# alexanderswerdlow/BEVGen

Measured on AMD Instinct MI355X. Metric: multi-view scenes/sec (6x256x256), higher is better.
Workload: dtype f32 (GEMM/conv/attention products as 3 f16 MFMAs on hi/lo splits, fp32 accumulate); 1 GPU; BASELINE configs[1]: Route M MaskGit, 6x256x256, batch 16 scenes/GPU, 18 iterations, + VQGAN decode to uint8; global_batch=16, parallelism=scene-parallel x1 (RCCL gather of uint8 pixels), precision_mode=f16x3

## Files before the change

### bevgen_amd/csrc/attention_split.hip

```cpp
#include <algorithm>

#include "common.h"
#include "kernels.h"
#include "profiler.h"

namespace bevgen {

typedef _Float16 half8 __attribute__((ext_vector_type(8)));
typedef _Float16 half4 __attribute__((ext_vector_type(4)));
typedef _Float16 half2v __attribute__((ext_vector_type(2)));
typedef uint32_t u32x4 __attribute__((ext_vector_type(4)));

constexpr int SKT = 32;
constexpr int SKLD = 72;
constexpr int SVLD = 36;
constexpr float kLo = 2048.f, kLoI = 1.f / 2048.f;
constexpr int PP_PLANE = SKT * SKLD;
static_assert(SKT * SKLD == 64 * SVLD, "K and V^T planes share one LDS stage layout");

#ifndef BEVGEN_ATTN_DIAG
#define BEVGEN_ATTN_DIAG 0
#endif
#ifndef BEVGEN_ATTN_BUF
#define BEVGEN_ATTN_BUF 1
#endif
#ifdef BEVGEN_ATTN_LAB
__device__ unsigned long long g_attn_trace[8 * 16 * 8];
#define PP_STAMP(k) do { if (TRACE && lane == 0 && t < 16) trace_lds[(wave * 16 + t) * 8 + (k)] = __builtin_readcyclecounter(); } while (0)
#else
#define PP_STAMP(k) do { } while (0)
#endif

template <bool TRACE, bool KS = false>
__global__ __launch_bounds__(512) void attention_split_kernel(AttnSplitArgs a) {
    __shared__ __attribute__((aligned(16))) _Float16 lds[2][4][PP_PLANE];
    __shared__ __attribute__((aligned(16))) float ostage[8][32 * 68];
#ifdef BEVGEN_ATTN_LAB
    __shared__ unsigned long long trace_lds[TRACE ? 8 * 16 * 8 : 1];
#endif

    const int tid = threadIdx.x, lane = tid & 63, wave = tid >> 6, grp = wave >> 2;
    const int qi = lane & 31, h = lane >> 5;
    const int nqb = gridDim.x, total = nqb * gridDim.y * gridDim.z;
    const int lin = blockIdx.x + nqb * (blockIdx.y + gridDim.y * blockIdx.z);
    const int vid = (total % 8 == 0) ? (lin % 8) * (total / 8) + lin / 8 : lin;
    const int qblk = vid % nqb, head = (vid / nqb) % gridDim.y, bz = vid / (nqb * gridDim.y);
    const int nks = KS ? a.ksplit : 1;
    const int b = KS ? bz / nks : bz, ks = KS ? bz - b * nks : 0;
    const int qrow = qblk * 256 + wave * 32 + qi;
    const bool qvalid = qrow < a.Nq;
    const int qc = qvalid ? qrow : a.Nq - 1;

    const long qoff = ((long)b * a.H + head) * a.Nq * 64 + (long)qc * 64 + 8 * h;
    const long koff = ((long)(b / a.kv_group) * a.H + head) * (long)a.Nk_pad * 64;
    const int bstep = a.bias_pk_tile_step;
    const int ntiles_all = a.Nk_pad / SKT;
    const int t_first = KS ? ks * ntiles_all / nks : 0;
    const int ntiles = KS ? (ks + 1) * ntiles_all / nks - t_first : ntiles_all;
    const float* Bp = a.bias_pk + (long)head * a.bias_head_stride + (long)(qblk * 8 + wave) * a.bias_pk_qb_stride + lane * 4 + (long)t_first * bstep;

    half8 qh[4], qs[4], qls[4];
#pragma unroll
    for (int s = 0; s < 4; ++s) {
        qh[s] = *reinterpret_cast<const half8*>(a.Qh + qoff + 16 * s);
        const half8 ql = *reinterpret_cast<const half8*>(a.Ql + qoff + 16 * s);
#pragma unroll
        for (int e = 0; e < 8; ++e) { qs[s][e] = qh[s][e] * (_Float16)kLoI; qls[s][e] = ql[e] * (_Float16)kLoI; }
    }
    f32x16 oM[2], oC[2];
#pragma unroll
    for (int t = 0; t < 2; ++t)
#pragma unroll
        for (int r = 0; r < 16; ++r) { oM[t][r] = 0.f; oC[t][r] = 0.f; }
    float m_run = kNegBig, l_run = 0.f;

    const int st = tid & 255;
    const _Float16 *src_hi, *src_lo;
    int src_step, dst_off;
    if (grp == 0) {
        const int kr = st >> 3, kc = st & 7;
        src_step = SKT * 64;
        src_hi = a.Kh + koff + kr * 64 + kc * 8 + (long)t_first * src_step; src_lo = a.Kl + koff + kr * 64 + kc * 8 + (long)t_first * src_step;
        dst_off = kr * SKLD + kc * 8;
    } else {
        const int vr = st >> 2, vc = st & 3;
        src_step = SKT;
        src_hi = a.VTh + koff + (long)vr * a.Nk_pad + vc * 8 + (long)t_first * src_step; src_lo = a.VTl + koff + (long)vr * a.Nk_pad + vc * 8 + (long)t_first * src_step;
        dst_off = 2 * PP_PLANE + vr * SVLD + vc * 8;
    }
    uint4 rh, rl;
    const int wave_u = __builtin_amdgcn_readfirstlane(wave);
    const int step_u = wave_u < 4 ? SKT * 64 : SKT;
    const _Float16* tb_hi = (wave_u < 4 ? a.Kh : a.VTh) + koff + (long)t_first * step_u;
    const _Float16* tb_lo = (wave_u < 4 ? a.Kl : a.VTl) + koff + (long)t_first * step_u;
    const __amdgpu_buffer_rsrc_t rs_hi = __builtin_amdgcn_make_buffer_rsrc(const_cast<_Float16*>(tb_hi), 0, -1, 0x00020000);
    const __amdgpu_buffer_rsrc_t rs_lo = __builtin_amdgcn_make_buffer_rsrc(const_cast<_Float16*>(tb_lo), 0, -1, 0x00020000);
    const int tv_off = wave_u < 4 ? ((st >> 3) * 64 + (st & 7) * 8) * 2 : ((st >> 2) * a.Nk_pad + (st & 3) * 8) * 2;
    auto gload = [&](int tile) {
        if (BEVGEN_ATTN_DIAG & (2 | 16)) return;
        if (BEVGEN_ATTN_BUF) {
            const int so = tile * step_u * 2;
            rh = __builtin_bit_cast(uint4, __builtin_amdgcn_raw_buffer_load_b128(rs_hi, tv_off, so, 0));
            rl = __builtin_bit_cast(uint4, __builtin_amdgcn_raw_buffer_load_b128(rs_lo, tv_off, so, 0));
            return;
        }
        rh = *reinterpret_cast<const uint4*>(src_hi + (long)tile * src_step);
        rl = *reinterpret_cast<const uint4*>(src_lo + (long)tile * src_step);
    };
    auto lstore = [&](int stage) {
        if (BEVGEN_ATTN_DIAG & (2 | 16)) return;
        uint2* dh = reinterpret_cast<uint2*>(&lds[stage][0][dst_off]);
        uint2* dl = reinterpret_cast<uint2*>(&lds[stage][1][dst_off]);
        dh[0] = make_uint2(rh.x, rh.y); dh[1] = make_uint2(rh.z, rh.w);
        dl[0] = make_uint2(rl.x, rl.y); dl[1] = make_uint2(rl.z, rl.w);
    };
    f32x16 bacc;
    if (BEVGEN_ATTN_DIAG) {
        for (int r = 0; r < 16; ++r) bacc[r] = (float)(lane + r);
        rh = make_uint4(lane, 1, 2, 3); rl = rh;
    }
    const float* Bu = a.bias_pk + (long)head * a.bias_head_stride + (long)(qblk * 8 + wave_u) * a.bias_pk_qb_stride + (long)t_first * bstep;
    const __amdgpu_buffer_rsrc_t rs_b = __builtin_amdgcn_make_buffer_rsrc(const_cast<float*>(Bu), 0, -1, 0x00020000);
    auto gload_bias = [&](int tile) {
        if (BEVGEN_ATTN_DIAG & (2 | 8)) return;
        if (BEVGEN_ATTN_BUF) {
            const int so = tile * bstep * 4;
#pragma unroll
            for (int g = 0; g < 4; ++g) {
                const u32x4 v = __builtin_amdgcn_raw_buffer_load_b128(rs_b, lane * 16, so + 1024 * g, 0);
                bacc[4 * g] = __uint_as_float(v.x); bacc[4 * g + 1] = __uint_as_float(v.y); bacc[4 * g + 2] = __uint_as_float(v.z); bacc[4 * g + 3] = __uint_as_float(v.w);
            }
            return;
        }
        const float* src = Bp + (long)tile * bstep;
#pragma unroll
        for (int g = 0; g < 4; ++g) {
            const float4 v = *reinterpret_cast<const float4*>(src + 256 * g);
            bacc[4 * g] = v.x; bacc[4 * g + 1] = v.y; bacc[4 * g + 2] = v.z; bacc[4 * g + 3] = v.w;
        }
    };

    gload_bias(0);
    gload(0);
    lstore(0);
    gload(min(1, ntiles - 1));
    __syncthreads();
    if (grp == 1) __syncthreads();

    f32x16 sM;
    half8 ph[2], pl[2];
    for (int t = 0; t <= ntiles; ++t) {
        PP_STAMP(0);
        if (t > 0 && !(BEVGEN_ATTN_DIAG & 4)) {
            const _Float16* Vh = &lds[(t - 1) & 1][2][0];
            const _Float16* Vl = &lds[(t - 1) & 1][3][0];
#pragma unroll
            for (int s = 0; s < 2; ++s) {
                half8 avh[2], avl[2];
#pragma unroll
                for (int u = 0; u < 2; ++u) {
                    const _Float16* vh = Vh + (32 * u + qi) * SVLD + 4 * h + 16 * s;
                    const _Float16* vl = Vl + (32 * u + qi) * SVLD + 4 * h + 16 * s;
                    const half4 h0 = *reinterpret_cast<const half4*>(vh), h1 = *reinterpret_cast<const half4*>(vh + 8);
                    const half4 l0 = *reinterpret_cast<const half4*>(vl), l1 = *reinterpret_cast<const half4*>(vl + 8);
                    avh[u] = half8{h0[0], h0[1], h0[2], h0[3], h1[0], h1[1], h1[2], h1[3]};
                    avl[u] = half8{l0[0], l0[1], l0[2], l0[3], l1[0], l1[1], l1[2], l1[3]};
                }
                oM[0] = __builtin_amdgcn_mfma_f32_32x32x16_f16(avh[0], ph[s], oM[0], 0, 0, 0);
                oM[1] = __builtin_amdgcn_mfma_f32_32x32x16_f16(avh[1], ph[s], oM[1], 0, 0, 0);
                oC[0] = __builtin_amdgcn_mfma_f32_32x32x16_f16(avl[0], ph[s], oC[0], 0, 0, 0);
                oC[1] = __builtin_amdgcn_mfma_f32_32x32x16_f16(avl[1], ph[s], oC[1], 0, 0, 0);
                oM[0] = __builtin_amdgcn_mfma_f32_32x32x16_f16(avh[0], pl[s], oM[0], 0, 0, 0);
                oM[1] = __builtin_amdgcn_mfma_f32_32x32x16_f16(avh[1], pl[s], oM[1], 0, 0, 0);
            }
        }
        if (t < ntiles && !(BEVGEN_ATTN_DIAG & 4)) {
            const _Float16* kh = &lds[t & 1][0][qi * SKLD + 8 * h];
            const _Float16* kl = &lds[t & 1][1][qi * SKLD + 8 * h];
#pragma unroll
            for (int s = 0; s < 4; ++s) {
                const half8 ah = *reinterpret_cast<const half8*>(kh + 16 * s);
                const half8 al = *reinterpret_cast<const half8*>(kl + 16 * s);
                if (s == 0) sM = __builtin_amdgcn_mfma_f32_32x32x16_f16(ah, qh[0], bacc, 0, 0, 0);
                else sM = __builtin_amdgcn_mfma_f32_32x32x16_f16(ah, qh[s], sM, 0, 0, 0);
                sM = __builtin_amdgcn_mfma_f32_32x32x16_f16(ah, qls[s], sM, 0, 0, 0);
                sM = __builtin_amdgcn_mfma_f32_32x32x16_f16(al, qs[s], sM, 0, 0, 0);
            }
        }
        if ((BEVGEN_ATTN_DIAG & 4) && t < ntiles) { for (int r = 0; r < 16; ++r) sM[r] = bacc[r] + (float)t; asm volatile("" : "+v"(sM)); }
        PP_STAMP(1);
        __syncthreads();

        PP_STAMP(2);
        lstore((t + 1) & 1);
        PP_STAMP(3);
        if (t < ntiles) {
#if BEVGEN_ATTN_DIAG & 1
            gload_bias(min(t + 1, ntiles - 1));
            gload(min(t + 2, ntiles - 1));
            const float m_new = m_run, alpha = 1.f, psum = 1.f;
#pragma unroll
            for (int s = 0; s < 2; ++s) {
                ph[s] = __builtin_bit_cast(half8, u32x4{__float_as_uint(sM[8 * s]), __float_as_uint(sM[8 * s + 1]), __float_as_uint(sM[8 * s + 2]), __float_as_uint(sM[8 * s + 3])});
                pl[s] = __builtin_bit_cast(half8, u32x4{__float_as_uint(sM[8 * s + 4]), __float_as_uint(sM[8 * s + 5]), __float_as_uint(sM[8 * s + 6]), __float_as_uint(sM[8 * s + 7])});
            }
#else
            float mx = kNegBig;
#pragma unroll
            for (int r = 0; r < 16; ++r) mx = fmaxf(mx, sM[r]);
            gload_bias(min(t + 1, ntiles - 1));
            __builtin_amdgcn_sched_barrier(0);
            mx = fmaxf(mx, xor32(mx));
            const float m_new = fmaxf(m_run, mx);
            const float alpha = __builtin_amdgcn_exp2f(m_run - m_new);
            PP_STAMP(6);
            float psum = 0.f;
            uint32_t hw[8], lw[8];
#pragma unroll
            for (int r = 0; r < 8; ++r) {
                const float p0 = __builtin_amdgcn_exp2f(sM[2 * r] - m_new), p1 = __builtin_amdgcn_exp2f(sM[2 * r + 1] - m_new);
                psum += p0;
                psum += p1;
                const half2v hp = {(_Float16)p0, (_Float16)p1};
                hw[r] = __builtin_bit_cast(uint32_t, hp);
                uint32_t l;
                asm("v_fma_mixlo_f16 %0, %1, 1.0, -%2 op_sel_hi:[0,0,1]" : "=v"(l) : "v"(p0), "v"(hw[r]));
                asm("v_fma_mixhi_f16 %0, %1, 1.0, -%2 op_sel:[0,0,1] op_sel_hi:[0,0,1]" : "+v"(l) : "v"(p1), "v"(hw[r]));
                lw[r] = l;
                if (r == 3) {
                    __builtin_amdgcn_sched_barrier(0);
                    gload(min(t + 2, ntiles - 1));
                    __builtin_amdgcn_sched_barrier(0);
                }
            }
#pragma unroll
            for (int s = 0; s < 2; ++s) {
                ph[s] = __builtin_bit_cast(half8, u32x4{hw[4 * s], hw[4 * s + 1], hw[4 * s + 2], hw[4 * s + 3]});
                pl[s] = __builtin_bit_cast(half8, u32x4{lw[4 * s], lw[4 * s + 1], lw[4 * s + 2], lw[4 * s + 3]});
            }
#endif
            PP_STAMP(7);
            l_run = l_run * alpha + psum;
            m_run = m_new;
            if (__builtin_amdgcn_ballot_w64(alpha != 1.f) != 0) {
#pragma unroll
                for (int u = 0; u < 2; ++u)
#pragma unroll
                    for (int r = 0; r < 16; ++r) { oM[u][r] *= alpha; oC[u][r] *= alpha; }
            }
        }
        PP_STAMP(4);
        __syncthreads();
        PP_STAMP(5);
    }
    if (grp == 0) __syncthreads();
#ifdef BEVGEN_ATTN_LAB
    if (TRACE && blockIdx.x == 1 && blockIdx.y == 3 && blockIdx.z == 5)
        for (int i = threadIdx.x; i < 8 * 16 * 8; i += 512) g_attn_trace[i] = trace_lds[i];
#endif

    const float l_tot = l_run + xor32(l_run);
    if (KS) {
        float* st = ostage[wave];
#pragma unroll
        for (int t = 0; t < 2; ++t)
#pragma unroll
            for (int g = 0; g < 4; ++g) {
                f32x4 o;
#pragma unroll
                for (int j = 0; j < 4; ++j) o[j] = oM[t][4 * g + j] + oC[t][4 * g + j] * kLoI;
                *reinterpret_cast<f32x4*>(st + qi * 68 + 32 * t + 8 * g + 4 * h) = o;
            }
        if (h == 0) *reinterpret_cast<float2*>(st + qi * 68 + 64) = make_float2(m_run, l_tot);
        const int c = lane & 15, rr = lane >> 4;
#pragma unroll
        for (int ps = 0; ps < 8; ++ps) {
            const int row = ps * 4 + rr, q = qblk * 256 + wave * 32 + row;
            const f32x4 v = *reinterpret_cast<const f32x4*>(st + row * 68 + 4 * c);
            if (q < a.Nq) {
                float* wrow = a.kws + ((((long)ks * a.B + b) * a.H + head) * a.Nq + q) * kAttnPartPitch;
                *reinterpret_cast<f32x4*>(wrow + 4 * c) = v;
                if (c == 0) *reinterpret_cast<float2*>(wrow + 64) = *reinterpret_cast<const float2*>(st + row * 68 + 64);
            }
        }
        return;
    }
    const float inv = 1.f / l_tot;
    if (!KS && a.Op) {
        float* st = ostage[wave];
#pragma unroll
        for (int t = 0; t < 2; ++t)
#pragma unroll
            for (int g = 0; g < 4; ++g) {
                f32x4 o;
#pragma unroll
                for (int j = 0; j < 4; ++j) o[j] = (oM[t][4 * g + j] + oC[t][4 * g + j] * kLoI) * inv;
                *reinterpret_cast<f32x4*>(st + qi * 68 + 32 * t + 8 * g + 4 * h) = o;
            }
        const int c = lane & 15, rr = lane >> 4;
        const int dsel = (c >> 3) * 32 + (c & 3) * 8;
        const bool lo_sel = (c >> 2) & 1;
        unsigned bad = 0;
#pragma unroll
        for (int ps = 0; ps < 8; ++ps) {
            const int row = ps * 4 + rr, q = qblk * 256 + wave * 32 + row;
            const f32x4 a0 = *reinterpret_cast<const f32x4*>(st + row * 68 + dsel);
            const f32x4 a1 = *reinterpret_cast<const f32x4*>(st + row * 68 + dsel + 4);
            half8 hi8, lo8;
#pragma unroll
            for (int e = 0; e < 4; ++e) {
                hi8[e] = split_hi(a0[e]); lo8[e] = split_lo(a0[e], hi8[e]);
                hi8[4 + e] = split_hi(a1[e]); lo8[4 + e] = split_lo(a1[e], hi8[4 + e]);
            }
            if (q < a.Nq) {
                if (!lo_sel) guard_half8(hi8, bad);
                *reinterpret_cast<half8*>(a.Op + ((long)b * a.Nq + q) * 2 * (a.H * 64) + head * 128 + c * 8) = lo_sel ? lo8 : hi8;
            }
        }
        if (bad) status_raise(a.status, BG_ST_F16_RANGE);
        return;
    }
    if (qvalid) {
        unsigned bad = 0;
        const long orow = (long)b * a.o_bstride + (long)qrow * a.o_qstride + (long)head * a.o_hstride;
#pragma unroll
        for (int t = 0; t < 2; ++t)
#pragma unroll
            for (int g = 0; g < 4; ++g) {
                const int d = 32 * t + 8 * g + 4 * h;
                float o[4];
#pragma unroll
                for (int j = 0; j < 4; ++j) o[j] = (oM[t][4 * g + j] + oC[t][4 * g + j] * kLoI) * inv;
                if (a.Op) store_planes4(a.Op + ((long)b * a.Nq + qrow) * 2 * (a.H * 64), head * 64 + d, make_float4(o[0], o[1], o[2], o[3]), bad);
                else *reinterpret_cast<float4*>(a.O + orow + d) = make_float4(o[0], o[1], o[2], o[3]);
            }
        if (bad) status_raise(a.status, BG_ST_F16_RANGE);
    }
}

__global__ __launch_bounds__(256) void pack_attn_bias_kernel(const float* __restrict__ bias, int ld, int Nq, int ntiles, float* __restrict__ out, long total4) {
    const long i = (long)blockIdx.x * 256 + threadIdx.x;
    if (i >= total4) return;
    const int lane = (int)(i & 63), g = (int)((i >> 6) & 3);
    const long t = i >> 8;
    const int tile = (int)(t % ntiles), qb = (int)(t / ntiles);
    const int q = min(32 * qb + (lane & 31), Nq - 1);
    reinterpret_cast<float4*>(out)[i] = *reinterpret_cast<const float4*>(bias + (long)q * ld + 32 * tile + 8 * g + 4 * (lane >> 5));
}
long attn_bias_packed_floats(int Nq, int Nk_pad) { return (long)cdiv(Nq, 256) * 8 * (Nk_pad / SKT) * 1024; }
void launch_pack_attn_bias(const float* bias, int ld, int Nq, int Nk_pad, float* out, hipStream_t s) {
    BG_REQUIRE(Nk_pad % SKT == 0 && Nk_pad > 0 && ld % 4 == 0 && ld >= Nk_pad, "pack_attn_bias: Nk_pad=%d ld=%d", Nk_pad, ld);
    const long total4 = attn_bias_packed_floats(Nq, Nk_pad) / 4;
    hipLaunchKernelGGL(pack_attn_bias_kernel, dim3((unsigned)cdiv(total4, 256L)), dim3(256), 0, s, bias, ld, Nq, Nk_pad / SKT, out, total4);
    LAUNCH_CHECK();
}

__device__ float g_zero_block[1024];
static const float* zero_block() {
    static const float* ptr[64] = {};
    int dev = 0;
    HIP_CHECK(hipGetDevice(&dev));
    if (!ptr[dev]) HIP_CHECK(hipGetSymbolAddress((void**)&ptr[dev], HIP_SYMBOL(g_zero_block)));
    return ptr[dev];
}

#ifdef BEVGEN_ATTN_LAB
}
#include "../../tools/attn_lab/attention_split_r1.inc"
namespace bevgen {
int g_attn_variant = 1;
void attn_lab_read_trace(unsigned long long* out) { HIP_CHECK(hipMemcpyFromSymbol(out, HIP_SYMBOL(g_attn_trace), sizeof(g_attn_trace))); }
#endif

__global__ __launch_bounds__(256) void attention_split_combine_kernel(AttnSplitArgs a) {
    const long i = (long)blockIdx.x * 256 + threadIdx.x;
    const long total = (long)a.B * a.H * a.Nq * 16;
    if (i >= total) return;
    const int d = (int)(i & 15) * 4;
    const long row = i >> 4;
    const int q = (int)(row % a.Nq), head = (int)((row / a.Nq) % a.H), b = (int)(row / ((long)a.Nq * a.H));
    const long stride = (long)a.B * a.H * a.Nq * kAttnPartPitch;
    const float* w0 = a.kws + row * kAttnPartPitch;
    float m = kNegBig;
    for (int k = 0; k < a.ksplit; ++k) m = fmaxf(m, w0[k * stride + 64]);
    float l = 0.f;
    float4 o = make_float4(0.f, 0.f, 0.f, 0.f);
    for (int k = 0; k < a.ksplit; ++k) {
        const float* w = w0 + k * stride;
        const float sc = __builtin_amdgcn_exp2f(w[64] - m);
        l = fmaf(w[65], sc, l);
        const float2 v0 = *reinterpret_cast<const float2*>(w + d), v1 = *reinterpret_cast<const float2*>(w + d + 2);
        o.x = fmaf(v0.x, sc, o.x); o.y = fmaf(v0.y, sc, o.y); o.z = fmaf(v1.x, sc, o.z); o.w = fmaf(v1.y, sc, o.w);
    }
    const float inv = 1.f / l;
    o.x *= inv; o.y *= inv; o.z *= inv; o.w *= inv;
    unsigned bad = 0;
    if (a.Op) store_planes4(a.Op + ((long)b * a.Nq + q) * 2 * (a.H * 64), head * 64 + d, o, bad);
    else *reinterpret_cast<float4*>(a.O + (long)b * a.o_bstride + (long)q * a.o_qstride + (long)head * a.o_hstride + d) = o;
    if (bad) status_raise(a.status, BG_ST_F16_RANGE);
}

void launch_attention_split(const AttnSplitArgs& a0, hipStream_t s) {
    AttnSplitArgs a = a0;
    a.status = status_current();
    if (a.ksplit < 1) a.ksplit = 1;
    BG_REQUIRE(a.ksplit == 1 || (a.kws && a.Nk_pad / SKT >= a.ksplit), "attention_split: key split %d needs a workspace and at least one key tile per range", a.ksplit);
    BG_REQUIRE(a.Nk_pad % SKT == 0 && a.Nk_pad > 0, "attention_split: Nk_pad=%d must be a positive multiple of %d", a.Nk_pad, SKT);
    a.bias_pk_tile_step = 1024;
    a.bias_pk_qb_stride = (long)(a.Nk_pad / SKT) * 1024;
    if (a.bias_pk == nullptr) {
        a.bias_pk = zero_block();
        a.bias_head_stride = 0; a.bias_pk_tile_step = 0; a.bias_pk_qb_stride = 0;
    }
    const dim3 grid(cdiv(a.Nq, 256), a.H, a.B * a.ksplit);
    ProfScope prof(PROF_ATTN, 4.0 * a.B * a.H * (double)a.Nq * a.Nk_pad * 64, s);
#ifdef BEVGEN_ATTN_LAB
    if (g_attn_variant == 0) launch_attention_split_r1(a, s);
    else if (g_attn_variant == 2) hipLaunchKernelGGL(attention_split_kernel<true>, grid, dim3(512), 0, s, a);
    else
#endif
    {
        if (a.ksplit > 1) hipLaunchKernelGGL((attention_split_kernel<false, true>), grid, dim3(512), 0, s, a);
        else hipLaunchKernelGGL((attention_split_kernel<false, false>), grid, dim3(512), 0, s, a);
    }
    LAUNCH_CHECK();
    if (a.ksplit > 1) {
        const long total = (long)a.B * a.H * a.Nq * 16;
        hipLaunchKernelGGL(attention_split_combine_kernel, dim3((unsigned)((total + 255) / 256)), dim3(256), 0, s, a);
        LAUNCH_CHECK();
    }
}

__global__ __launch_bounds__(256) void attn_split_operands_kernel(const float* __restrict__ q, const float* __restrict__ k, const float* __restrict__ v, _Float16* __restrict__ Qh,
                                                                 _Float16* __restrict__ Ql, _Float16* __restrict__ Kh, _Float16* __restrict__ Kl, _Float16* __restrict__ VTh,
                                                                 _Float16* __restrict__ VTl, long nq, long nk, int Nk_pad, float qmul, unsigned* __restrict__ status) {
    const long i = (long)blockIdx.x * 256 + threadIdx.x;
    unsigned bad = 0;
    if (i < nq) {
        const float x = q[i] * qmul;
        const _Float16 hi = (_Float16)x;
        guard_half(hi, bad);
        Qh[i] = hi; Ql[i] = (_Float16)((x - (float)hi) * kLo);
    }
    if (i < nk) {
        const float x = k[i];
        const _Float16 hi = (_Float16)x;
        guard_half(hi, bad);
        Kh[i] = hi; Kl[i] = (_Float16)((x - (float)hi) * kLo);
        const long bh = i / ((long)Nk_pad * 64), r = i % ((long)Nk_pad * 64);
        const int j = (int)(r / 64), d = (int)(r % 64);
        const float y = v[i];
        const _Float16 vh = (_Float16)y;
        guard_half(vh, bad);
        const long dst = bh * (long)Nk_pad * 64 + (long)d * Nk_pad + j;
        VTh[dst] = vh; VTl[dst] = (_Float16)((y - (float)vh) * kLo);
    }
    if (bad) status_raise(status, BG_ST_F16_RANGE);
}
void launch_attn_split_operands(const float* q, const float* k, const float* v, void* Qh, void* Ql, void* Kh, void* Kl, void* VTh, void* VTl, int B, int H, int Nq, int Nk_pad,
                                float qmul, hipStream_t s) {
    const long nq = (long)B * H * Nq * 64, nk = (long)B * H * Nk_pad * 64;
    hipLaunchKernelGGL(attn_split_operands_kernel, dim3((unsigned)cdiv(std::max(nq, nk), 256L)), dim3(256), 0, s, q, k, v, reinterpret_cast<_Float16*>(Qh), reinterpret_cast<_Float16*>(Ql),
                       reinterpret_cast<_Float16*>(Kh), reinterpret_cast<_Float16*>(Kl), reinterpret_cast<_Float16*>(VTh), reinterpret_cast<_Float16*>(VTl), nq, nk, Nk_pad, qmul, status_current());
    LAUNCH_CHECK();
}

__device__ __forceinline__ void split1(float v, _Float16& hi, _Float16& lo, unsigned& bad) {
    hi = (_Float16)v;
    lo = (_Float16)((v - (float)hi) * kLo);
    guard_half(hi, bad);
}

__global__ __launch_bounds__(256) void muse_q_prep_split_kernel(const float* __restrict__ qraw, const float* __restrict__ q_scale, _Float16* __restrict__ Qh,
                                                                _Float16* __restrict__ Ql, int H, int Nq, long total, float post, unsigned* __restrict__ status) {
    const int lane = threadIdx.x & 63;
    const long w = (long)blockIdx.x * 4 + (threadIdx.x >> 6);
    if (w >= total) return;
    const int h = (int)(w % H);
    const long bn = w / H;
    const int n = (int)(bn % Nq);
    const long b = bn / Nq;
    const float v = qraw[bn * (H * 64) + h * 64 + lane] * 8.0f;
    const float nrm = fmaxf(sqrtf(wave_sum(v * v)), 1e-12f);
    const float q = ((v / nrm) * q_scale[lane]) * post;
    _Float16 hi, lo;
    unsigned bad = 0;
    split1(q, hi, lo, bad);
    const long dst = ((b * H + h) * Nq + n) * 64 + lane;
    Qh[dst] = hi;
    Ql[dst] = lo;
    if (bad) status_raise(status, BG_ST_F16_RANGE);
}

void launch_muse_q_prep_split(const float* qraw, const float* q_scale, void* Qh, void* Ql, int B, int H, int Nq, float post, hipStream_t s) {
    const long total = (long)B * Nq * H;
    hipLaunchKernelGGL(muse_q_prep_split_kernel, dim3((int)((total + 3) / 4)), dim3(256), 0, s, qraw, q_scale, reinterpret_cast<_Float16*>(Qh),
                       reinterpret_cast<_Float16*>(Ql), H, Nq, total, post, status_current());
    LAUNCH_CHECK();
}

__global__ __launch_bounds__(256) void muse_kv_prep_split_kernel(const float* __restrict__ kvraw, const float* __restrict__ null_kv, const float* __restrict__ k_scale,
                                                                 _Float16* __restrict__ Kh, _Float16* __restrict__ Kl, _Float16* __restrict__ VTh,
                                                                 _Float16* __restrict__ VTl, int H, int Nk, int Nk_pad, unsigned* __restrict__ status) {
    __shared__ float vt[64][65];
    unsigned bad = 0;
    const int lane = threadIdx.x & 63, wv = threadIdx.x >> 6;
    const int j0 = blockIdx.x * 64, h = blockIdx.y;
    const long b = blockIdx.z;
    const long kbase = (b * H + h) * (long)Nk_pad * 64;
    for (int jj = wv; jj < 64; jj += 4) {
        const int j = j0 + jj;
        float kv = 0.f, vv = 0.f;
        if (j <= Nk) {
            if (j == 0) {
                kv = null_kv[h * 64 + lane];
                vv = null_kv[(long)H * 64 + h * 64 + lane];
            } else {
                const float* src = kvraw + (b * Nk + (j - 1)) * (2L * H * 64);
                kv = src[h * 64 + lane];
                vv = src[H * 64 + h * 64 + lane];
            }
            const float nrm = fmaxf(sqrtf(wave_sum(kv * kv)), 1e-12f);
            const float k = (kv / nrm) * k_scale[lane];
            _Float16 hi, lo;
            split1(k, hi, lo, bad);
            Kh[kbase + (long)j * 64 + lane] = hi;
            Kl[kbase + (long)j * 64 + lane] = lo;
        }
        vt[jj][lane] = vv;
    }
    __syncthreads();
    for (int d = wv; d < 64; d += 4) {
        const int j = j0 + lane;
        if (j < Nk_pad) {
            _Float16 hi, lo;
            split1(vt[lane][d], hi, lo, bad);
            VTh[kbase + (long)d * Nk_pad + j] = hi;
            VTl[kbase + (long)d * Nk_pad + j] = lo;
        }
    }
    if (bad) status_raise(status, BG_ST_F16_RANGE);
}

__global__ __launch_bounds__(64) void muse_null_kv_prep_kernel(const float* __restrict__ null_kv, const float* __restrict__ k_scale, _Float16* __restrict__ out, int H,
                                                               unsigned* __restrict__ status) {
    const int h = blockIdx.x, lane = threadIdx.x;
    const float kv = null_kv[h * 64 + lane], vv = null_kv[(long)H * 64 + h * 64 + lane];
    const float nrm = fmaxf(sqrtf(wave_sum(kv * kv)), 1e-12f);
    const float k = (kv / nrm) * k_scale[lane];
    _Float16 hi, lo;
    unsigned bad = 0;
    split1(k, hi, lo, bad);
    out[h * 64 + lane] = hi;
    out[H * 64 + h * 64 + lane] = lo;
    split1(vv, hi, lo, bad);
    out[2 * H * 64 + h * 64 + lane] = hi;
    out[3 * H * 64 + h * 64 + lane] = lo;
    if (bad) status_raise(status, BG_ST_F16_RANGE);
}
void launch_muse_null_kv_prep(const float* null_kv, const float* k_scale, void* out, int H, hipStream_t s) {
    hipLaunchKernelGGL(muse_null_kv_prep_kernel, dim3(H), dim3(64), 0, s, null_kv, k_scale, reinterpret_cast<_Float16*>(out), H, status_current());
    LAUNCH_CHECK();
}

void launch_muse_kv_prep_split(const float* kvraw, const float* null_kv, const float* k_scale, void* Kh, void* Kl, void* VTh, void* VTl, int B, int H, int Nk,
                               int Nk_pad, hipStream_t s) {
    dim3 grid(cdiv(Nk_pad, 64), H, B);
    hipLaunchKernelGGL(muse_kv_prep_split_kernel, grid, dim3(256), 0, s, kvraw, null_kv, k_scale, reinterpret_cast<_Float16*>(Kh), reinterpret_cast<_Float16*>(Kl),
                       reinterpret_cast<_Float16*>(VTh), reinterpret_cast<_Float16*>(VTl), H, Nk, Nk_pad, status_current());
    LAUNCH_CHECK();
}

}
```

### bevgen_amd/csrc/kernels.h

```cpp
#pragma once
#include <hip/hip_runtime.h>
#include <stdint.h>

namespace bevgen {

enum { MODE_PLAIN = 0, MODE_CONV3 = 1, MODE_CONV3S = 2 };
enum { ACT_NONE = 0, ACT_GELU = 1 };
enum { EPI_PLAIN = 0, EPI_MUSE_Q = 1, EPI_GEGLU = 2, EPI_MUSE_KV = 3, EPI_MUSE_QKV = 4 };

struct GemmArgs {
    const float* A = nullptr;
    const float* B = nullptr;
    float* C = nullptr;
    const float* R = nullptr;
    const float* bias_n = nullptr;
    const float* bias_m = nullptr;
    int M = 0, N = 0, K = 0;
    int lda = 0, ldb = 0, ldc = 0, ldr = 0;
    int batch = 1;
    long strideA = 0, strideB = 0, strideC = 0, strideR = 0;
    float alpha = 1.f;
    int act = ACT_NONE;
    int mode = MODE_PLAIN;
    int conv_h = 0, conv_w = 0, conv_cin = 0, conv_up = 0;
    int conv_hin = 0, conv_win = 0, conv_stride = 0, conv_pad = -1;
    const uint16_t* B_hi = nullptr;
    const uint16_t* B_lo = nullptr;
    bool b_lo_zero = false;
    const uint16_t* A_hi = nullptr;
    const uint16_t* A_lo = nullptr;
    const void* zero_page = nullptr;
    int epi = 0;
    const float* epi_scale = nullptr;
    void* epi_hi = nullptr;
    void* epi_lo = nullptr;
    int epi_rows = 0, epi_heads = 0;
    void* epi_hi2 = nullptr;
    void* epi_lo2 = nullptr;
    const void* epi_aux = nullptr;
    int epi_ld = 0;
    float epi_post = 1.f;
    float* gn_part = nullptr;
    void* epi_qh = nullptr;
    void* epi_ql = nullptr;
    const float* epi_qscale = nullptr;
    int ksplit = 1;
    float* kpart = nullptr;
    int a_bytes = 0;
    bool conv_general = false;
    int tile_band = 0;
    int m_base = 0;
    bool no_row_split = false;
    int force_wm = 0;
    unsigned* status = nullptr;
    bool row_major_epi = false;
    bool r_prefetch = false;
    void* ln_out_planes = nullptr;
    float* ln_out_stats = nullptr;
    int ln_out_ld = 0;
    const float* ln_in_stats = nullptr;
    const float* ln_in_gsums = nullptr;
    int ln_in_groups = 0, ln_in_count = 0;
    float ln_eps = 1e-5f;
    const float* ln_in_cs = nullptr;
    void* sk_ws = nullptr;
    unsigned sk_epoch = 0;
    int sk_tiles = 0;
    bool sk_force = false;
    int ln_rows = 0;
};
void launch_ln_stats_finalize(const float* group_sums, float* row_stats, int rows, int groups, int count, float eps, hipStream_t s);
void launch_ln_fold_weight(const float* W, const float* gamma, float* Wg, float* cs, int N, int K, int Kg, hipStream_t s);
void launch_gemm(const GemmArgs& g, hipStream_t stream);
void launch_gemm_split_glds(const GemmArgs& g, hipStream_t stream);
bool xcd_placement_verified();
size_t gemm_sk_ws_bytes();
bool gemm_sk_pays(long rows, int N, int K);

struct SplitPlanes { const uint16_t* hi; const uint16_t* lo; bool lo_zero = false;  };
void launch_gemm_split(const GemmArgs& g, hipStream_t stream);
void launch_split_weight(const float* w, void* planes , long n, hipStream_t s);
void split_registry_set(const void* table );

int gemm_skinny_ksplit(int M, int N, int K);
size_t gemm_skinny_ws_bytes(int M, int N, int K);
void launch_gemm_skinny_ws(const GemmArgs& g, float* ws, hipStream_t stream);

void launch_layernorm(const float* x, int ldx, const float* gamma, const float* beta, float* y, int ldy, int rows, int D, float eps, hipStream_t s);
void launch_geglu_layernorm(const float* h, int ldh, const float* gamma, float* y, int ldy, int rows, int F, float eps, hipStream_t s);
void launch_layernorm_planes(const float* x, int ldx, const float* gamma, const float* beta, void* planes, int ldy, int rows, int D, float eps, hipStream_t s);
void launch_geglu_layernorm_planes(const float* h, int ldh, const float* gamma, void* planes, int ldy, int rows, int F, float eps, hipStream_t s);
size_t groupnorm_ws_bytes(int n, int hw);
bool vq_out_conv_supported(int C, int cout);
void launch_vq_out_conv(const float* x, const float* stats, const float* gamma, const float* beta, const float* wgt, const float* bias, const float* mean, const float* stdv, int clamp01,
                        float* y, uint8_t* y8, int n, int H, int W, int C, int cout, hipStream_t s);
void launch_groupnorm_stats(const float* x, float* stats, void* ws , int n, int hw, int C, float eps, hipStream_t s);
bool groupnorm_partials_supported(int hw, int C);
size_t groupnorm_part_floats(int n, int hw, int C);
void launch_groupnorm_stats_from_partials(const float* part, float* stats, int n, int hw, int C, float eps, hipStream_t s);
void launch_groupnorm_apply(const float* x, const float* stats, const float* gamma, const float* beta, float* y, int n, int hw, int C, int do_swish, hipStream_t s);
void launch_to_planes(const float* x, void* planes, int n, int hw, int C, hipStream_t s);
void launch_groupnorm_apply_planes(const float* x, const float* stats, const float* gamma, const float* beta, void* planes, int n, int hw, int C, int do_swish, hipStream_t s);

struct AttnArgs {
    const float* Q; const float* K; const float* V; const float* bias; const float* R; float* O;
    int B, H, Nq, Nk_pad;
    long q_bstride, q_hstride;
    long kv_bstride, kv_hstride;
    int ldbias; long bias_head_stride;
    float scale;
    long o_bstride, o_qstride, o_hstride;
    int kv_group = 1;
    const uint16_t* tiles = nullptr; long tiles_head_stride = 0; int tiles_ld = 0;
};
void launch_attention(const AttnArgs& a, hipStream_t s);
size_t attn_tiles_elems(int heads, int Nq, int Nk_pad);
void launch_build_attn_tiles(const float* masked_bias, long bias_head_stride, int ldbias, int heads, int Nq, int Nk_pad, uint16_t* tiles, hipStream_t s);
void launch_splitk_reduce(const GemmArgs& g, const float* partial, int ksplit, hipStream_t s);

constexpr float kLog2e = 1.44269504088896340736f;
struct AttnSplitArgs {
    const _Float16 *Qh, *Ql, *Kh, *Kl, *VTh, *VTl;
    const float* bias;
    float* O;
    int B, H, Nq, Nk_pad;
    int ldbias; long bias_head_stride;
    float scale;
    long o_bstride, o_qstride, o_hstride;
    _Float16* Op;
    const float* bias_pk = nullptr;
    int bias_pk_tile_step = 0;
    long bias_pk_qb_stride = 0;
    int kv_group = 1;
    int ksplit = 1;
    float* kws = nullptr;
    unsigned* status = nullptr;
};
constexpr int kAttnPartPitch = 68;
inline long attn_split_ws_floats(int B, int H, int Nq, int ksplit) { return (long)ksplit * B * H * Nq * kAttnPartPitch; }
long attn_bias_packed_floats(int Nq, int Nk_pad);
void launch_pack_attn_bias(const float* bias, int ld, int Nq, int Nk_pad, float* out, hipStream_t s);
void launch_attn_split_operands(const float* q, const float* k, const float* v, void* Qh, void* Ql, void* Kh, void* Kl, void* VTh, void* VTl, int B, int H, int Nq, int Nk_pad,
                                float qmul, hipStream_t s);
void launch_attention_split(const AttnSplitArgs& a, hipStream_t s);
void launch_muse_q_prep_split(const float* qraw, const float* q_scale, void* Qh, void* Ql, int B, int H, int Nq, float post, hipStream_t s);
void launch_muse_null_kv_prep(const float* null_kv, const float* k_scale, void* out , int H, hipStream_t s);
void launch_muse_kv_prep_split(const float* kvraw, const float* null_kv, const float* k_scale, void* Kh, void* Kl, void* VTh, void* VTl, int B, int H, int Nk,
                               int Nk_pad, hipStream_t s);

struct SparseVis {
    const uint8_t* allowed = nullptr; int ldallowed = 0; long allowed_head_stride = 0;
    const uint8_t* lay = nullptr; long lay_head_stride = 0; int nb = 0, blk = 1;
    const uint16_t* chunks = nullptr; long chunks_head_stride = 0; int chunks_ld = 0;
    int has_allowed = 0, has_lay = 0, has_chunks = 0;
};
inline SparseVis vis_fix(SparseVis v, const void* any_valid) {
    v.has_allowed = v.allowed != nullptr; v.has_lay = v.lay != nullptr; v.has_chunks = v.chunks != nullptr;
    if (!v.allowed) { v.allowed = reinterpret_cast<const uint8_t*>(any_valid); v.ldallowed = 0; v.allowed_head_stride = 0; }
    if (!v.lay) { v.lay = reinterpret_cast<const uint8_t*>(any_valid); v.lay_head_stride = 0; v.nb = 0; v.blk = 1 << 30; }
    if (!v.chunks) { v.chunks = reinterpret_cast<const uint16_t*>(any_valid); v.chunks_head_stride = 0; v.chunks_ld = 0; }
    return v;
}

struct DecodeAttnArgs {
    const float* q = nullptr;
    int ldq = 0;
    const void* kcache = nullptr;
    const void* vcache = nullptr;
    const float* bias = nullptr;
    int ldbias = 0;
    SparseVis vis;
    const float* append_k = nullptr;
    const float* append_v = nullptr;
    const float* R = nullptr;
    float* O = nullptr;
    int ldr = 0, ldo = 0;
    int B = 0, H = 0;
    int n = 0;
    const int* d_n = nullptr;
    int n_hint = 0;
    int Lmax = 0;
    float scale = 1.f;
    int kv_dtype = 0;
    int shared_prefix = 0;
    int group = 1;
    unsigned* status = nullptr;
};
int decode_attention_splits(int B, int H, int n_max);
size_t decode_attention_ws_bytes(int B, int H, int S);
void launch_decode_attention_ws(const DecodeAttnArgs& a, float* ws, int S, hipStream_t s);
void launch_decode_attention_combine(const DecodeAttnArgs& a, const float* ws, int S, hipStream_t s);

struct RowSrc {
    const float* base = nullptr; int ld = 0;
    const float* partial = nullptr; int ns = 0; long pstride = 0; int pld = 0;
    const float* bias = nullptr;
    int has_bias = 0;
};
void launch_rowsrc_materialize(const RowSrc& r, float* out, int M, int D, int* counter , hipStream_t s);

struct ArAttnFusedArgs {
    RowSrc x;
    const float *ln_w = nullptr, *ln_b = nullptr; float eps = 1e-5f;
    const float* qkv = nullptr;
    const float* xn = nullptr;
    const float* wqkv = nullptr;
    const void* wqkv_h = nullptr;
    const float* bqkv = nullptr;
    const float *ln_cs = nullptr, *ln_ds = nullptr;
    void* kcache = nullptr;
    void* vcache = nullptr;
    int kv_dtype = 0;
    const float* bias = nullptr; int ldbias = 0;
    SparseVis vis;
    float* out = nullptr; int ldo = 0;
    int B = 0, G = 1, H = 0, D = 0, Lmax = 0, Lpad = 0;
    int n = 0; const int* d_n = nullptr; int n_hint = 0;
    int prefix = 0;
    float scale = 0.125f;
    long long* trace = nullptr;
    int ksplit = 1;
    float* kws = nullptr;
    int stage_cap = -1;
    int has_bias = 0;
    unsigned* status = nullptr;
};
bool ar_attn_fused_supported(int B, int G, int D, int H);
void launch_ar_ln_fold(const float* W, const float* b, const float* gamma, const float* beta, float* cs, float* ds, int N, int K, hipStream_t s);
void launch_ar_attn_fused(const ArAttnFusedArgs& a, hipStream_t s);

struct SkinnyFusedArgs {
    const float* A = nullptr; int lda = 0;
    const RowSrc* a_src = nullptr;
    float* xn_out = nullptr; int ldxn = 0;
    const float *ln_w = nullptr, *ln_b = nullptr; float eps = 1e-5f;
    const float *ln_cs = nullptr, *ln_ds = nullptr;
    const float* Wp = nullptr;
    int w_f16 = 0;
    const float* bias = nullptr;
    float* C = nullptr; int ldc = 0;
    int M = 0, N = 0, K = 0, ksplit = 0 , act = 0;
    long long* trace = nullptr;
    int has_ln_b = 0;
    RowSrc src;
};
struct MlpFusedArgs {
    const float* A = nullptr; int lda = 0;
    const float* ln_w = nullptr;
    const float *ln_cs = nullptr, *ln_ds = nullptr;
    float eps = 1e-5f;
    const float* Wup = nullptr;
    const float* Wdn = nullptr;
    int w_f16 = 0;
    float* hidden = nullptr;
    float* C = nullptr;
    unsigned* sync = nullptr;
    unsigned* err = nullptr;
    int M = 0, D = 0;
    long long* trace = nullptr;
    int acq = 1;
};
constexpr int MLP_FUSED_PLANES = 8;
size_t mlp_fused_sync_words();
bool mlp_fused_supported(int M, int D, bool w_f16);
void launch_ar_mlp_fused(const MlpFusedArgs& g, hipStream_t s);
size_t skinny_packed_floats(int N, int K);
void launch_pack_skinny_weight(const float* W, float* Wp, int N, int K, hipStream_t s);
void launch_pack_skinny_weight_f16(const float* W, void* Wp , int N, int K, hipStream_t s);
int skinny_fused_ksplit(int N, int K);
bool skinny_fused_supported(int M, int N, int K, bool ln);
bool skinny_fused_f16_ok(int N, int K, bool ln);
size_t ar_attn_fused_lds_bytes(int G, int D, int Lpad);
size_t ar_attn_fused_max_lds();
size_t ar_attn_lds_bytes(int G, int Lpad);
void launch_skinny_fused(const SkinnyFusedArgs& g, hipStream_t s);

void launch_camera_embed(const float* I_inv, const float* E_inv, const float* plane , const float* Wimg, const float* Wcam,
                         float* img , float* c_embed , int B, int C, int T, int D, hipStream_t s);
void launch_cond_embed(const int64_t* cond_ids, const float* cond_tok, const float* cond_pos, const float* bev_grid ,
                       const float* Wbev, const float* bbev, const float* bev_cam_pos , const float* c_embed ,
                       float* out, int B, int C, int K, int D, int cond_vocab, hipStream_t s);
void launch_token_embed(const int64_t* ids, const float* tok_emb, const float* img , const float* pos, float* x,
                        int B, int N, int D, int vocab_rows, hipStream_t s);

void launch_muse_q_prep(const float* qraw, const float* q_scale, float* Q, int B, int H, int Nq, hipStream_t s);
void launch_muse_kv_prep(const float* kvraw, const float* null_kv , const float* k_scale, float* K, float* V,
                         int B, int H, int Nk, int Nk_pad, hipStream_t s);
void launch_ar_qkv_scatter(const float* qkv, float* Q , void* kcache, void* vcache, int kv_dtype,
                           int B, int H, int n, int pos0, int Lmax, hipStream_t s);
void launch_ar_kv_append(const float* qkv, void* kcache, void* vcache, int kv_dtype, int B, int H, int pos0, const int* d_pos, int Lmax, hipStream_t s);

void launch_remask(int64_t* ids, const float* scores, const int64_t* init_ids , int rows, int T, int n_mask, int64_t mask_id, hipStream_t s);
void launch_maskgit_pick(int64_t* ids, const float* logits, int ldl, const float* gumbel_u , int rows, int V, int k, float temperature,
                         int64_t mask_id, hipStream_t s, unsigned long long seed = 0 , unsigned iter = 0,
                         float* conf_scores = nullptr, int conf_mode = 0 );
void launch_critic_scores(const float* embed, int lde, const float* w, const float* b, const float* u , float noise_scale, float frac,
                          float* scores, int rows, int D, hipStream_t s, unsigned long long seed = 0, unsigned iter = 0);
void launch_philox_fill(float* out, long n, unsigned long long seed, unsigned iter, unsigned stream, int V , hipStream_t s);
struct ArPickTail {
    int64_t* out_all = nullptr; const int64_t* fwd_idx = nullptr; int N = 0;
    const float *tok_emb = nullptr, *img_embed = nullptr, *pos_emb = nullptr; float* x = nullptr; int C = 0, T = 0, D = 0, vocab_rows = 0;
};
void launch_ar_pick(const float* logits, int ldl, const float* u , const int* d_step , const int64_t* forced,
                    int64_t* out, int rows, int V, int top_k, float temperature, hipStream_t s, const ArPickTail* tail = nullptr);

void launch_ar_score_rows(const float* logits, int ldl, const int64_t* target , const float* weight, const int64_t* fwd_idx, int b, int s0, int rows,
                          int N, int V, float* nll, float* wnll, hipStream_t s);
void launch_mean_fixed_order(const float* x, long n, float* out, hipStream_t s);

void launch_codebook_gather(const int64_t* ids, const float* codebook, float* out, int rows, int dim, int n_embed, hipStream_t s);
void launch_nhwc_to_nchw(const float* x, float* y, int n, int hw, int C, int ldc, const float* mean, const float* stdv, int clamp01, hipStream_t s,
                         uint8_t* y8 = nullptr );
void launch_nchw_to_nhwc(const float* x, float* y, int n, int hw, int C, hipStream_t s);
void launch_range_exponent(const float* x, long elems , unsigned* amax, int* e, hipStream_t s);
void launch_range_split(const float* x, void* planes, long pixels, int C, const int* e, hipStream_t s);
void launch_range_scale(const float* x, float* y, long elems, const int* e, hipStream_t s);
void launch_range_unscale(float* y, const float* bias, const float* residual, long rows, int C, const int* e, float* gn_part, hipStream_t s);
void launch_row_softmax(float* x, int rows, int cols, float scale, hipStream_t s, int ld = 0 );

void launch_fill(float* p, long n, float v, hipStream_t s);
void launch_add(const float* a, const float* b, float* c, long n, hipStream_t s);
void launch_scale(float* p, long n, float v, hipStream_t s);

}
```

### bevgen_amd/csrc/muse.cpp

```cpp
#include "model.h"

namespace bevgen {

namespace {

struct MuseWs {
    int B = 0;
    int S = 1;

    long rows = 0;
    float *img = nullptr, *c_embed = nullptr, *context = nullptr;
    std::vector<float*> crossK, crossV;
    float *x = nullptr, *xn = nullptr, *qraw = nullptr, *kvraw = nullptr, *Q = nullptr, *Ks = nullptr, *Vs = nullptr, *att = nullptr, *h = nullptr, *g = nullptr;
    float* attn_ws = nullptr; int attn_ks = 1;
    float* kpart = nullptr;
    float *stats_d = nullptr, *stats_f = nullptr;
    float* rowstat = nullptr;
    void* sk_ws = nullptr;
    unsigned sk_epoch = 0;
};

int ln_fold_level(const Ctx& c, long rows) {
    const char* e = getenv("BEVGEN_LN_FOLD");
    const int env = e ? atoi(e) : 1;
    (void)rows;
    if (c.muse.empty() || !c.muse[0].fold_w4) return 0;
    return std::max(0, std::min(env, 2));
}

constexpr int KSPLIT_MAX = 6;
constexpr long kSkMaxRows = 8192;
int ksplit_env() { static const int v = getenv("BEVGEN_KSPLIT") ? atoi(getenv("BEVGEN_KSPLIT")) : 0; return v; }
int pick_ksplit(long rows, int N, int K) {
    if ((long)cdiv(rows, 256) * cdiv(N, 128) >= 256) return 1;
    const long tiles = (long)cdiv(rows, 128) * cdiv(N, 128);
    if (tiles >= 160) return 1;
    int s = (K >= 2048 && tiles > 128) ? 2 : 1;
    if (ksplit_env() > 0) s = std::min(KSPLIT_MAX, ksplit_env());
    while (s > 1 && K / 32 < 2 * s) --s;
    return s;
}

int pick_attn_ksplit(long blocks, int ntiles) {
    static const int env = getenv("BEVGEN_ATTN_KSPLIT") ? atoi(getenv("BEVGEN_ATTN_KSPLIT")) : 0;
    if (env > 0) return std::max(1, std::min(std::min(env, 8), ntiles));
    if (blocks * 2 > 256) return 1;
    const int ks = std::min(std::min(4, (int)(256 / blocks)), ntiles / 8);
    return std::max(ks, 1);
}

size_t muse_ws_bytes(const Ctx& c, int B) {
    const size_t rows = (size_t)B * c.N;
    const size_t crows = (size_t)B * c.K;
    size_t f = 0;
    f += rows * c.D * 2;
    f += (size_t)B * c.cfg.num_cams * c.D + crows * c.D;
    f += (size_t)c.cfg.num_layers * 2 * B * c.H * c.NkC_pad * 64 + (size_t)B * c.K * 2 + (size_t)B * c.cfg.num_cams * c.D;
    f += rows * c.D * 3;
    f += std::max(rows, crows) * 2 * c.D;
    f += rows * c.D;
    f += (size_t)2 * B * c.H * c.NkS_pad * 64;
    f += rows * 2 * c.F + rows * c.Fpad;
    f += rows * (c.V + 1);
    if (std::max(pick_ksplit((long)rows, c.D, c.D), pick_ksplit((long)rows, c.D, c.Fpad)) > 1) f += (size_t)KSPLIT_MAX * rows * c.D;
    {
        const int ks = pick_attn_ksplit((long)cdiv(c.N, 256) * c.H * B, c.NkS_pad / 32);
        if (ks > 1) f += (size_t)attn_split_ws_floats(B, c.H, c.N, ks);
    }
    f += rows * (size_t)(2 * (c.D / 32) + 2 * (c.Fpad / 32) + 4);
    return f * sizeof(float) + (64 + 4 * c.cfg.num_layers) * 256 + (rows <= kSkMaxRows ? gemm_sk_ws_bytes() + 256 : 0);
}

void gemm(const float* A, int lda, const float* W, int ldb, float* C, int ldc, int M, int N, int K, const float* R, int ldr, hipStream_t s) {
    GemmArgs g;
    g.A = A; g.B = W; g.C = C; g.R = R;
    g.M = M; g.N = N; g.K = K;
    g.lda = lda; g.ldb = ldb; g.ldc = ldc; g.ldr = ldr;
    launch_gemm(g, s);
}

struct LnFold {
    const float* in_stats = nullptr; const float* in_cs = nullptr;
    const float* in_gsums = nullptr; int in_groups = 0, in_count = 0;
    void* out_planes = nullptr; float* out_stats = nullptr; int out_ld = 0;
};
void set_sk(GemmArgs& g, MuseWs* w);
void set_fold(GemmArgs& g, const LnFold* f, int rows) {
    if (!f) return;
    g.ln_in_stats = f->in_stats; g.ln_in_cs = f->in_cs;
    g.ln_in_gsums = f->in_gsums; g.ln_in_groups = f->in_groups; g.ln_in_count = f->in_count;
    g.ln_out_planes = f->out_planes; g.ln_out_stats = f->out_stats; g.ln_out_ld = f->out_ld;
    g.ln_rows = rows;
}

void gemm_planes(const void* Aplanes, int lda, const float* W, int ldb, float* C, int ldc, int M, int N, int K, const float* R, int ldr, hipStream_t s, float* kpart = nullptr,
                 const LnFold* fold = nullptr, MuseWs* sk = nullptr) {
    GemmArgs g;
    g.A_hi = reinterpret_cast<const uint16_t*>(Aplanes); g.A_lo = g.A_hi + 32;
    g.B = W; g.C = C; g.R = R;
    g.M = M; g.N = N; g.K = K;
    g.lda = lda; g.ldb = ldb; g.ldc = ldc; g.ldr = ldr;
    const bool use_sk = sk && gemm_sk_pays(M, N, K);
    if (kpart && N <= 1024 && !fold && !use_sk) { g.ksplit = pick_ksplit(M, N, K); g.kpart = kpart; }
    set_fold(g, fold, M);
    if (use_sk) set_sk(g, sk);
    launch_gemm(g, s);
}

void gemm_planes_q(const void* Aplanes, int lda, const float* W, const float* q_scale, void* Qh, void* Ql, int B, int H, int Nq, int D, hipStream_t s, float* kpart = nullptr,
                   float* qraw = nullptr, const LnFold* fold = nullptr, MuseWs* sk = nullptr) {
    const bool use_sk = sk && gemm_sk_pays((long)B * Nq, H * 64, D);
    if (!fold && !use_sk && kpart && qraw && H * 64 <= 1024 && pick_ksplit((long)B * Nq, H * 64, D) > 1) {
        gemm_planes(Aplanes, lda, W, D, qraw, H * 64, B * Nq, H * 64, D, nullptr, 0, s, kpart);
        launch_muse_q_prep_split(qraw, q_scale, Qh, Ql, B, H, Nq, 8.0f * kLog2e, s);
        return;
    }
    GemmArgs g;
    g.A_hi = reinterpret_cast<const uint16_t*>(Aplanes); g.A_lo = g.A_hi + 32;
    g.B = W;
    g.M = B * Nq; g.N = H * 64; g.K = D;
    g.lda = lda; g.ldb = D; g.ldc = H * 64;
    g.epi = EPI_MUSE_Q; g.epi_scale = q_scale; g.epi_hi = Qh; g.epi_lo = Ql; g.epi_rows = Nq; g.epi_heads = H;
    g.epi_post = 8.0f * kLog2e;
    set_fold(g, fold, B * Nq);
    if (use_sk) set_sk(g, sk);
    launch_gemm(g, s);
}

void set_sk(GemmArgs& g, MuseWs* w) {
    if (!w || !w->sk_ws) return;
    g.sk_ws = w->sk_ws;
    g.sk_epoch = ++w->sk_epoch;
}

void muse_prepare(Ctx& c, MuseWs& w, const int64_t* cond, const float* I_inv, const float* E_inv, int B, hipStream_t s, int samples_per_layout = 1) {
    const auto& g = c.cfg;
    const std::string p = "transformer.";
    const int S = samples_per_layout < 1 ? 1 : samples_per_layout;
    BG_REQUIRE(B % S == 0, "batch %d is not a multiple of samples_per_layout %d", B, S);
    const int G = B / S;
    w.S = S;
    w.B = B;
    w.rows = (long)B * c.N;
    Arena& a = c.arena;
    a.reserve(muse_ws_bytes(c, B));
    a.reset();
    const int D = c.D, H = c.H;
    w.img = g.image_embed ? a.get<float>((size_t)w.rows * D) : nullptr;
    w.c_embed = g.image_embed ? a.get<float>((size_t)B * g.num_cams * D) : nullptr;
    w.context = a.get<float>((size_t)G * c.K * D);
    w.x = a.get<float>((size_t)w.rows * D);
    w.xn = a.get<float>((size_t)w.rows * D);
    w.qraw = a.get<float>((size_t)w.rows * D);
    w.att = a.get<float>((size_t)w.rows * D);
    w.kvraw = a.get<float>((size_t)std::max<long>(w.rows, (long)B * c.K) * 2 * D);
    w.Q = a.get<float>((size_t)w.rows * D);
    const size_t kvS = (size_t)B * H * c.NkS_pad * 64;
    w.Ks = a.get<float>(kvS);
    w.Vs = a.get<float>(kvS);
    w.h = a.get<float>((size_t)w.rows * 2 * c.F);
    w.g = a.get<float>((size_t)w.rows * c.Fpad);
    w.kpart = std::max(pick_ksplit(w.rows, D, D), pick_ksplit(w.rows, D, c.Fpad)) > 1 ? a.get<float>((size_t)KSPLIT_MAX * w.rows * D) : nullptr;
    w.attn_ks = pick_attn_ksplit((long)cdiv(c.N, 256) * H * B, c.NkS_pad / 32);
    w.attn_ws = w.attn_ks > 1 ? a.get<float>((size_t)attn_split_ws_floats(B, H, c.N, w.attn_ks)) : nullptr;
    w.stats_d = a.get<float>((size_t)w.rows * 2 * (D / 32));
    w.stats_f = a.get<float>((size_t)w.rows * 2 * (c.Fpad / 32));
    w.rowstat = a.get<float>((size_t)w.rows * 2);
    w.sk_ws = nullptr;
    if (w.rows <= kSkMaxRows && g.precision == BEVGEN_PRECISION_F16X3) {
        w.sk_ws = a.alloc(gemm_sk_ws_bytes());
        HIP_CHECK(hipMemsetAsync(w.sk_ws, 0, 1024 * sizeof(unsigned), s));
        w.sk_epoch = 0;
    }
    HIP_CHECK(hipMemsetAsync(w.Ks, 0, kvS * sizeof(float), s));
    HIP_CHECK(hipMemsetAsync(w.Vs, 0, kvS * sizeof(float), s));

    if (g.image_embed)
        launch_camera_embed(I_inv, E_inv, c.image_plane, c.pf(p + "img_embed.weight"), c.pf(p + "cam_embed.weight"), w.img, w.c_embed, B, g.num_cams, c.T, D, s);
    const int64_t* cond_g = cond;
    const float* c_embed_g = w.c_embed;
    if (S > 1) {
        int64_t* cg = a.get<int64_t>((size_t)G * c.K);
        HIP_CHECK(hipMemcpy2DAsync(cg, (size_t)c.K * 8, cond, (size_t)S * c.K * 8, (size_t)c.K * 8, G, hipMemcpyDeviceToDevice, s));
        cond_g = cg;
        if (w.c_embed) {
            float* eg = a.get<float>((size_t)G * g.num_cams * D);
            HIP_CHECK(hipMemcpy2DAsync(eg, (size_t)g.num_cams * D * 4, w.c_embed, (size_t)S * g.num_cams * D * 4, (size_t)g.num_cams * D * 4, G, hipMemcpyDeviceToDevice, s));
            c_embed_g = eg;
        }
    }
    launch_cond_embed(cond_g, c.pf(p + "cond_token_emb.weight"), c.pf(p + "cond_pos_emb.weight"), g.bev_embed ? c.pf(p + "bev_grid") : nullptr,
                      g.bev_embed ? c.pf(p + "bev_embed.weight") : nullptr, g.bev_embed ? c.pf(p + "bev_embed.bias") : nullptr,
                      g.bev_embed ? c.pf(p + "bev_cam_pos_emb") : nullptr, c_embed_g, w.context, G, g.num_cams, c.K, D, g.cond_vocab_size, s);

    const size_t kvC = (size_t)G * H * c.NkC_pad * 64;
    w.crossK.resize(g.num_layers);
    w.crossV.resize(g.num_layers);
    for (int i = 0; i < g.num_layers; ++i) {
        w.crossK[i] = a.get<float>(kvC);
        w.crossV[i] = a.get<float>(kvC);
        HIP_CHECK(hipMemsetAsync(w.crossK[i], 0, kvC * sizeof(float), s));
        HIP_CHECK(hipMemsetAsync(w.crossV[i], 0, kvC * sizeof(float), s));
        const MuseLayer& l = c.muse[i];
        gemm(w.context, D, l.to_kv[1], D, w.kvraw, 2 * D, G * c.K, 2 * D, D, nullptr, 0, s);
        if (c.cfg.precision == BEVGEN_PRECISION_F16X3) {
            _Float16* kh = reinterpret_cast<_Float16*>(w.crossK[i]);
            _Float16* vh = reinterpret_cast<_Float16*>(w.crossV[i]);
            launch_muse_kv_prep_split(w.kvraw, l.null_kv[1], l.k_scale[1], kh, kh + kvC, vh, vh + kvC, G, H, c.K, c.NkC_pad, s);
        } else {
            launch_muse_kv_prep(w.kvraw, l.null_kv[1], l.k_scale[1], w.crossK[i], w.crossV[i], G, H, c.K, c.NkC_pad, s);
        }
    }
}

void muse_blocks(Ctx& c, MuseWs& w, const int64_t* ids, hipStream_t s) {
    const auto& g = c.cfg;
    const std::string p = "transformer.";
    const int D = c.D, H = c.H, B = w.B, N = c.N;
    const int rows = (int)w.rows;
    launch_token_embed(ids, c.pf(p + "token_emb.weight"), w.img, c.pf(p + "pos_emb.weight"), w.x, B, N, D, g.vocab_size + 1, s);
    const bool split = g.precision == BEVGEN_PRECISION_F16X3;
    const int fold = split ? ln_fold_level(c, rows) : 0;
    bool x_planes_ready = false;
    const char* merge_env = getenv("BEVGEN_LN_MERGE");
    const bool tile_merge = merge_env ? merge_env[0] == 't' : rows <= 3072;
    auto consumer = [&](const float* gsums, int groups, int count, const float* cs) {
        LnFold f;
        f.in_cs = cs;
        if (tile_merge) { f.in_gsums = gsums; f.in_groups = groups; f.in_count = count; }
        else { launch_ln_stats_finalize(gsums, w.rowstat, rows, groups, count, 1e-5f, s); f.in_stats = w.rowstat; }
        return f;
    };
    LnFold prod_x;
    prod_x.out_planes = w.xn; prod_x.out_stats = w.stats_d; prod_x.out_ld = D;
    for (int i = 0; i < g.num_layers; ++i) {
        const MuseLayer& l = c.muse[i];
        if (split) {
            const bool f0 = fold == 2 && x_planes_ready;
            LnFold cons_x;
            if (!f0) launch_layernorm_planes(w.x, D, l.norm_g[0], nullptr, w.xn, D, rows, D, 1e-5f, s);
            else cons_x = consumer(w.stats_d, D / 32, D, nullptr);
            static const int qkv_merge = getenv("BEVGEN_QKV_MERGE") ? atoi(getenv("BEVGEN_QKV_MERGE")) : 1;
            const bool merged = l.to_qkv_self && qkv_merge != 0 && (qkv_merge != 3 || rows <= 3072);
            if (!merged) {
                cons_x.in_cs = l.fold_q_self_cs;
                gemm_planes_q(w.xn, D, f0 ? l.fold_q_self : l.to_q[0], l.q_scale[0], w.Q, reinterpret_cast<_Float16*>(w.Q) + (size_t)rows * D, B, H, N, D, s, w.kpart, w.qraw,
                              f0 ? &cons_x : nullptr, &w);
            }
            {
                const size_t kvS_ = (size_t)B * H * c.NkS_pad * 64;
                _Float16 *Kp = reinterpret_cast<_Float16*>(w.Ks), *Vp = reinterpret_cast<_Float16*>(w.Vs);
                GemmArgs gk;
                gk.A_hi = reinterpret_cast<const uint16_t*>(w.xn); gk.A_lo = gk.A_hi + 32;
                gk.B = merged ? (f0 ? l.fold_qkv : l.to_qkv_self) : (f0 ? l.fold_kv_self : l.to_kv[0]);
                gk.M = rows; gk.N = (merged ? 3 : 2) * D; gk.K = D; gk.lda = D; gk.ldb = D; gk.ldc = gk.N;
                gk.epi = merged ? EPI_MUSE_QKV : EPI_MUSE_KV;
                gk.epi_scale = l.k_scale[0]; gk.epi_hi = Kp; gk.epi_lo = Kp + kvS_; gk.epi_hi2 = Vp; gk.epi_lo2 = Vp + kvS_;
                gk.epi_aux = l.null_self; gk.epi_rows = N; gk.epi_heads = H; gk.epi_ld = c.NkS_pad;
                if (merged) {
                    gk.epi_qh = w.Q; gk.epi_ql = reinterpret_cast<_Float16*>(w.Q) + (size_t)rows * D; gk.epi_qscale = l.q_scale[0];
                    gk.epi_post = 8.0f * kLog2e;
                }
                if (f0) { cons_x.in_cs = merged ? l.fold_qkv_cs : l.fold_kv_self_cs; set_fold(gk, &cons_x, rows); }
                static const int qkv_wm4 = getenv("BEVGEN_QKV_WM4") ? atoi(getenv("BEVGEN_QKV_WM4")) : 1;
                if (qkv_wm4 && merged) gk.force_wm = 4;
                if (gemm_sk_pays(rows, gk.N, gk.K)) set_sk(gk, &w);
                launch_gemm(gk, s);
            }
        } else {
            launch_layernorm(w.x, D, l.norm_g[0], nullptr, w.xn, D, rows, D, 1e-5f, s);
            gemm(w.xn, D, l.to_q[0], D, w.qraw, D, rows, D, D, nullptr, 0, s);
            gemm(w.xn, D, l.to_kv[0], D, w.kvraw, 2 * D, rows, 2 * D, D, nullptr, 0, s);
        }
        const size_t qN = (size_t)rows * D, kvS = (size_t)B * H * c.NkS_pad * 64, kvC = (size_t)(B / w.S) * H * c.NkC_pad * 64;
        _Float16 *Qh = reinterpret_cast<_Float16*>(w.Q), *Ksh = reinterpret_cast<_Float16*>(w.Ks), *VTsh = reinterpret_cast<_Float16*>(w.Vs);
        AttnSplitArgs sa{};
        if (split) {
            sa.Qh = Qh; sa.Ql = Qh + qN; sa.Kh = Ksh; sa.Kl = Ksh + kvS; sa.VTh = VTsh; sa.VTl = VTsh + kvS;
            sa.bias = c.bias_self; sa.bias_pk = c.bias_self_pk; sa.O = w.att; sa.B = B; sa.H = H; sa.Nq = N; sa.Nk_pad = c.NkS_pad;
            sa.ldbias = c.ldS; sa.bias_head_stride = 0; sa.scale = 8.0f * kLog2e;
            sa.o_bstride = (long)N * D; sa.o_qstride = D; sa.o_hstride = 64;
            sa.Op = reinterpret_cast<_Float16*>(w.att);
            sa.ksplit = w.attn_ks; sa.kws = w.attn_ws;
            launch_attention_split(sa, s);
            sa.ksplit = 1; sa.kws = nullptr;
        } else {
            launch_muse_q_prep(w.qraw, l.q_scale[0], w.Q, B, H, N, s);
            launch_muse_kv_prep(w.kvraw, l.null_kv[0], l.k_scale[0], w.Ks, w.Vs, B, H, N, c.NkS_pad, s);
        }
        AttnArgs a{};
        a.Q = w.Q; a.K = w.Ks; a.V = w.Vs; a.bias = c.bias_self; a.R = nullptr; a.O = w.att;
        a.B = B; a.H = H; a.Nq = N; a.Nk_pad = c.NkS_pad;
        a.q_bstride = (long)H * N * 64; a.q_hstride = (long)N * 64;
        a.kv_bstride = (long)H * c.NkS_pad * 64; a.kv_hstride = (long)c.NkS_pad * 64;
        a.ldbias = c.ldS; a.bias_head_stride = 0; a.scale = 8.0f;
        a.o_bstride = (long)N * D; a.o_qstride = D; a.o_hstride = 64;
        if (!split) launch_attention(a, s);
        if (split) gemm_planes(w.att, D, l.to_out[0], D, w.x, D, rows, D, D, w.x, D, s, w.kpart, fold == 2 ? &prod_x : nullptr, &w);
        else gemm(w.att, D, l.to_out[0], D, w.x, D, rows, D, D, w.x, D, s);
        if (split) {
            LnFold cons_x;
            if (fold != 2) launch_layernorm_planes(w.x, D, l.norm_g[1], nullptr, w.xn, D, rows, D, 1e-5f, s);
            else cons_x = consumer(w.stats_d, D / 32, D, l.fold_q_cross_cs);
            gemm_planes_q(w.xn, D, fold == 2 ? l.fold_q_cross : l.to_q[1], l.q_scale[1], w.Q, reinterpret_cast<_Float16*>(w.Q) + (size_t)rows * D, B, H, N, D, s, w.kpart, w.qraw,
                          fold == 2 ? &cons_x : nullptr, &w);
        } else {
            launch_layernorm(w.x, D, l.norm_g[1], nullptr, w.xn, D, rows, D, 1e-5f, s);
            gemm(w.xn, D, l.to_q[1], D, w.qraw, D, rows, D, D, nullptr, 0, s);
        }
        if (split) {
            _Float16 *ckh = reinterpret_cast<_Float16*>(w.crossK[i]), *cvh = reinterpret_cast<_Float16*>(w.crossV[i]);
            sa.Kh = ckh; sa.Kl = ckh + kvC; sa.VTh = cvh; sa.VTl = cvh + kvC;
            sa.bias = c.bias_cross; sa.bias_pk = c.bias_cross_pk; sa.Nk_pad = c.NkC_pad; sa.ldbias = c.ldC;
            sa.kv_group = w.S;
            launch_attention_split(sa, s);
        } else {
            launch_muse_q_prep(w.qraw, l.q_scale[1], w.Q, B, H, N, s);
            a.K = w.crossK[i]; a.V = w.crossV[i]; a.bias = c.bias_cross; a.Nk_pad = c.NkC_pad;
            a.kv_bstride = (long)H * c.NkC_pad * 64; a.kv_hstride = (long)c.NkC_pad * 64;
            a.ldbias = c.ldC;
            a.kv_group = w.S;
            launch_attention(a, s);
        }
        if (split) {
            gemm_planes(w.att, D, l.to_out[1], D, w.x, D, rows, D, D, w.x, D, s, w.kpart, fold == 2 ? &prod_x : nullptr, &w);
            if (fold != 2) launch_layernorm_planes(w.x, D, l.ff_g0, nullptr, w.xn, D, rows, D, 1e-5f, s);
            if (l.ff_w1_geglu) {
                GemmArgs ge;
                ge.A_hi = reinterpret_cast<const uint16_t*>(w.xn); ge.A_lo = ge.A_hi + 32;
                ge.B = fold == 2 ? l.fold_w1 : l.ff_w1_geglu; ge.C = w.h;
                ge.M = rows; ge.N = 2 * c.Fpad; ge.K = D;
                ge.lda = D; ge.ldb = D; ge.ldc = c.Fpad;
                ge.epi = EPI_GEGLU;
                LnFold fg;
                if (fold == 2) fg = consumer(w.stats_d, D / 32, D, l.fold_w1_cs);
                if (fold >= 1) { fg.out_planes = w.g; fg.out_stats = w.stats_f; fg.out_ld = c.Fpad; }
                if (fold >= 1) set_fold(ge, &fg, rows);
                if (gemm_sk_pays(rows, ge.N, ge.K)) set_sk(ge, &w);
                launch_gemm(ge, s);
                if (fold == 0) launch_layernorm_planes(w.h, c.Fpad, l.ff_g3, nullptr, w.g, c.Fpad, rows, c.F, 1e-5f, s);
            } else {
                gemm_planes(w.xn, D, l.ff_w1, D, w.h, 2 * c.F, rows, 2 * c.F, D, nullptr, 0, s);
                launch_geglu_layernorm_planes(w.h, 2 * c.F, l.ff_g3, w.g, c.Fpad, rows, c.F, 1e-5f, s);
            }
            LnFold fd;
            if (fold >= 1 && l.ff_w1_geglu) fd = consumer(w.stats_f, c.Fpad / 32, c.F, l.fold_w4_cs);
            const bool prod_next = fold == 2 && i + 1 < g.num_layers;
            if (prod_next) { fd.out_planes = w.xn; fd.out_stats = w.stats_d; fd.out_ld = D; }
            const bool cons = fd.in_stats || fd.in_gsums, any = cons || fd.out_planes;
            gemm_planes(w.g, c.Fpad, cons ? l.fold_w4 : l.ff_w4_padded, c.Fpad, w.x, D, rows, D, c.Fpad, w.x, D, s, w.kpart, any ? &fd : nullptr, &w);
            x_planes_ready = prod_next;
        } else {
            gemm(w.att, D, l.to_out[1], D, w.x, D, rows, D, D, w.x, D, s);
            launch_layernorm(w.x, D, l.ff_g0, nullptr, w.xn, D, rows, D, 1e-5f, s);
            gemm(w.xn, D, l.ff_w1, D, w.h, 2 * c.F, rows, 2 * c.F, D, nullptr, 0, s);
            launch_geglu_layernorm(w.h, 2 * c.F, l.ff_g3, w.g, c.Fpad, rows, c.F, 1e-5f, s);
            gemm(w.g, c.Fpad, l.ff_w4_padded, c.Fpad, w.x, D, rows, D, c.Fpad, w.x, D, s);
        }
    }
    launch_layernorm(w.x, D, c.pf(p + "transformer_blocks.norm.gamma"), nullptr, w.xn, D, rows, D, 1e-5f, s);
}

}

void muse_forward(Ctx& c, const int64_t* ids, const int64_t* cond, const float* I_inv, const float* E_inv, int B, float* logits, float* embed, hipStream_t s) {
    BG_REQUIRE(c.cfg.route == BEVGEN_ROUTE_MASKGIT, "context was not created for the MaskGit route");
    BG_REQUIRE(B >= 1, "batch must be positive");
    MuseWs w;
    muse_prepare(c, w, cond, I_inv, E_inv, B, s);
    muse_blocks(c, w, ids, s);
    const int rows = (int)w.rows;
    if (embed) HIP_CHECK(hipMemcpyAsync(embed, w.xn, (size_t)rows * c.D * sizeof(float), hipMemcpyDeviceToDevice, s));
    if (logits) gemm(w.xn, c.D, c.pf("transformer.to_logits.weight"), c.D, logits, c.V, rows, c.V, c.D, nullptr, 0, s);
}

void maskgit_generate(Ctx& c, const int64_t* cond, const float* I_inv, const float* E_inv, int B, int timesteps, const int32_t* sched, float temperature,
                      int topk_k, float critic_noise_scale, const float* gumbel_u, const float* critic_u, const int64_t* init_ids, int64_t* out, hipStream_t s,
                      unsigned long long noise_seed, int score_mode, int samples_per_layout) {
    BG_REQUIRE(c.cfg.route == BEVGEN_ROUTE_MASKGIT, "context was not created for the MaskGit route");
    BG_REQUIRE(B >= 1 && timesteps >= 1 && sched, "bad generate arguments");
    BG_REQUIRE(score_mode != 0 || c.find("token_critic.to_pred.weight"), "maskgit_generate: the context holds no token critic (token_critic.to_pred.*): use score_mode 1 / 2");
    BG_REQUIRE(score_mode >= 0 && score_mode <= 2, "score_mode %d: 0 token critic, 1 softmax confidence, 2 softmax confidence with re-masking of earlier tokens", score_mode);
    MuseWs w;
    muse_prepare(c, w, cond, I_inv, E_inv, B, s, samples_per_layout);
    const int rows = (int)w.rows;
    const int seqs = B * c.cfg.num_cams;
    const int T = c.T, V = c.V, D = c.D;
    float* logits = c.arena.get<float>((size_t)rows * V);
    float* scores = c.arena.get<float>((size_t)rows);
    const int64_t mask_id = c.cfg.vocab_size;
    int64_t* ids = out;
    launch_fill_i64(ids, rows, mask_id, s);
    launch_fill(scores, rows, 0.f, s);
    for (int step = 0; step < timesteps; ++step) {
        const int steps_until_x0 = timesteps - 1 - step;
        const double frac = (double)steps_until_x0 / (double)timesteps;
        launch_remask(ids, scores, init_ids, seqs, T, sched[step], mask_id, s);
        muse_blocks(c, w, ids, s);
        gemm(w.xn, D, c.pf("transformer.to_logits.weight"), D, logits, V, rows, V, D, nullptr, 0, s);
        launch_maskgit_pick(ids, logits, V, gumbel_u ? gumbel_u + (size_t)step * rows * V : nullptr, rows, V, topk_k, (float)((double)temperature * frac), mask_id, s,
                            noise_seed, (unsigned)step, score_mode ? scores : nullptr, score_mode);
        if (score_mode == 0 && step + 1 < timesteps) {
            muse_blocks(c, w, ids, s);
            launch_critic_scores(w.xn, D, c.pf("token_critic.to_pred.weight"), c.pf("token_critic.to_pred.bias"),
                                 critic_u ? critic_u + (size_t)step * rows : nullptr, critic_noise_scale, (float)frac, scores, rows, D, s, noise_seed, (unsigned)step);
        }
    }
}

}
```

### bevgen_amd/csrc/sampler.hip

```cpp
#include "common.h"
#include "kernels.h"

namespace bevgen {

constexpr int VPL_MAX = 16;

__device__ __forceinline__ uint32_t ordered_key(float x) {
    const uint32_t u = __float_as_uint(x);
    return (u & 0x80000000u) ? ~u : (u | 0x80000000u);
}

__device__ __forceinline__ uint32_t kth_largest_key(const uint32_t (&key)[VPL_MAX], const bool (&valid)[VPL_MAX], int k) {
    uint32_t t = 0;
    for (int bit = 31; bit >= 0; --bit) {
        const uint32_t cand = t | (1u << bit);
        int cnt = 0;
#pragma unroll
        for (int j = 0; j < VPL_MAX; ++j) cnt += (valid[j] && key[j] >= cand) ? 1 : 0;
#pragma unroll
        for (int o = 32; o > 0; o >>= 1) cnt += __shfl_xor(cnt, o, 64);
        if (cnt >= k) t = cand;
    }
    return t;
}

__device__ __forceinline__ void wave_argmax(float& v, int& idx) {
#pragma unroll
    for (int o = 32; o > 0; o >>= 1) {
        const float ov = __shfl_xor(v, o, 64);
        const int oi = __shfl_xor(idx, o, 64);
        if (ov > v || (ov == v && oi < idx)) { v = ov; idx = oi; }
    }
}

__global__ __launch_bounds__(256) void remask_kernel(int64_t* __restrict__ ids, const float* __restrict__ scores, const int64_t* __restrict__ init_ids,
                                                     int T, int n_mask, int64_t mask_id) {
    extern __shared__ float sc[];
    const int row = blockIdx.x;
    for (int i = threadIdx.x; i < T; i += blockDim.x) sc[i] = scores[(long)row * T + i];
    __syncthreads();
    for (int i = threadIdx.x; i < T; i += blockDim.x) {
        const float s = sc[i];
        int rank = 0;
        for (int j = 0; j < T; ++j) rank += (sc[j] > s || (sc[j] == s && j < i)) ? 1 : 0;
        int64_t v = ids[(long)row * T + i];
        if (rank < n_mask) v = mask_id;
        if (init_ids) {
            const int64_t iv = init_ids[(long)row * T + i];
            if (iv != mask_id) v = iv;
        }
        ids[(long)row * T + i] = v;
    }
}

void launch_remask(int64_t* ids, const float* scores, const int64_t* init_ids, int rows, int T, int n_mask, int64_t mask_id, hipStream_t s) {
    BG_REQUIRE(T >= 1 && (size_t)T * sizeof(float) <= 64 * 1024, "remask: %d scores per row do not fit the 64 KiB of dynamic LDS", T);
    hipLaunchKernelGGL(remask_kernel, dim3(rows), dim3(256), T * sizeof(float), s, ids, scores, init_ids, T, n_mask, mask_id);
    LAUNCH_CHECK();
}

__global__ __launch_bounds__(256) void maskgit_pick_kernel(int64_t* __restrict__ ids, const float* __restrict__ logits, int ldl, const float* __restrict__ gumbel_u,
                                                           long rows, int V, int k, float temp_div, int64_t mask_id, unsigned long long seed, unsigned iter,
                                                           float* __restrict__ conf_scores, int conf_mode, unsigned* __restrict__ status) {
    const int lane = threadIdx.x & 63;
    const long row = (long)blockIdx.x * 4 + (threadIdx.x >> 6);
    if (row >= rows) return;
    const bool was_mask = ids[row] == mask_id;
    if (!was_mask) {
        if (conf_mode == 1 && lane == 0) conf_scores[row] = -1e5f;
        if (conf_mode != 2) return;
    }
    const float* lr = logits + row * ldl;
    float x[VPL_MAX];
    uint32_t key[VPL_MAX];
    bool valid[VPL_MAX];
#pragma unroll
    for (int j = 0; j < VPL_MAX; ++j) {
        const int i = lane + 64 * j;
        valid[j] = i < V;
        x[j] = valid[j] ? lr[i] : 0.f;
        key[j] = ordered_key(x[j]);
    }
    {
        bool nf = false;
#pragma unroll
        for (int j = 0; j < VPL_MAX; ++j) nf |= nonfinite(x[j]);
        if (nf) status_raise(status, BG_ST_NONFINITE_LOGITS);
    }
    const bool noisy = gumbel_u != nullptr || seed != 0;
    uint32_t thr = 0;
    if (noisy) thr = kth_largest_key(key, valid, k);
    float best = -INFINITY;
    int bidx = 0x7fffffff;
    Philox4 ph{};
#pragma unroll
    for (int j = 0; j < VPL_MAX; ++j) {
        const int i = lane + 64 * j;
        if (!valid[j]) continue;
        if (!gumbel_u && seed && (j & 3) == 0) ph = philox4(seed, (unsigned long long)(row * V + lane + 256 * (j >> 2)), iter, 0u);
        if (key[j] < thr) continue;
        float v = x[j] / temp_div;
        if (noisy) {
            const float u = gumbel_u ? gumbel_u[row * V + i] : philox_to_unit(ph.v[j & 3]);
            const float l1 = logf(fmaxf(u, 1e-20f));
            v += -logf(fmaxf(-l1, 1e-20f));
        }
        if (v > best || (v == best && i < bidx)) { best = v; bidx = i; }
    }
    wave_argmax(best, bidx);
    if (lane == 0 && was_mask) ids[row] = bidx;
    if (conf_mode) {
        float mx = -INFINITY;
#pragma unroll
        for (int j = 0; j < VPL_MAX; ++j)
            if (valid[j]) mx = fmaxf(mx, x[j]);
        mx = wave_max(mx);
        float sum = 0.f, xp = 0.f;
#pragma unroll
        for (int j = 0; j < VPL_MAX; ++j) {
            if (!valid[j]) continue;
            sum += expf(x[j] - mx);
            if (lane + 64 * j == bidx) xp = x[j];
        }
        sum = wave_sum(sum);
        xp = wave_sum(xp);
        if (lane == 0) conf_scores[row] = 1.f - expf(xp - mx) / sum;
    }
}

void launch_maskgit_pick(int64_t* ids, const float* logits, int ldl, const float* gumbel_u, int rows, int V, int k, float temperature, int64_t mask_id, hipStream_t s,
                         unsigned long long seed, unsigned iter, float* conf_scores, int conf_mode) {
    BG_REQUIRE(V <= 64 * VPL_MAX, "maskgit_pick: vocabulary %d > %d", V, 64 * VPL_MAX);
    BG_REQUIRE(k >= 1, "maskgit_pick: top-k count %d < 1 (topk_filter_thres = 1 keeps no logit)", k);
    BG_REQUIRE(conf_mode == 0 || conf_scores, "maskgit_pick: confidence scores requested without an output buffer");
    const float temp_div = fmaxf(temperature, 1e-10f);
    hipLaunchKernelGGL(maskgit_pick_kernel, dim3(cdiv(rows, 4)), dim3(256), 0, s, ids, logits, ldl, gumbel_u, (long)rows, V, k, temp_div, mask_id, seed, iter, conf_scores,
                       conf_mode, status_current());
    LAUNCH_CHECK();
}

__global__ __launch_bounds__(256) void critic_scores_kernel(const float* __restrict__ embed, int lde, const float* __restrict__ w, const float* __restrict__ b,
                                                            const float* __restrict__ u, float noise_scale, float frac, float* __restrict__ scores, long rows, int D,
                                                            unsigned long long seed, unsigned iter, unsigned* __restrict__ status) {
    const int lane = threadIdx.x & 63;
    const long row = (long)blockIdx.x * 4 + (threadIdx.x >> 6);
    if (row >= rows) return;
    const float* e = embed + row * lde;
    float acc = 0.f;
    for (int i = lane * 4; i < D; i += 256) {
        const float4 ev = *reinterpret_cast<const float4*>(e + i);
        const float4 wv = *reinterpret_cast<const float4*>(w + i);
        acc = fmaf(ev.x, wv.x, acc); acc = fmaf(ev.y, wv.y, acc); acc = fmaf(ev.z, wv.z, acc); acc = fmaf(ev.w, wv.w, acc);
    }
    acc = wave_sum(acc);
    if (lane == 0) {
        float sc = acc + b[0];
        const float uu = u ? u[row] : (seed ? philox_uniform(seed, (unsigned long long)row, iter, 1u) : 0.5f);
        sc += ((uu - 0.5f) * noise_scale) * frac;
        if (nonfinite(sc)) status_raise(status, BG_ST_NONFINITE_LOGITS);
        scores[row] = sc;
    }
}

void launch_critic_scores(const float* embed, int lde, const float* w, const float* b, const float* u, float noise_scale, float frac, float* scores, int rows, int D, hipStream_t s,
                          unsigned long long seed, unsigned iter) {
    BG_REQUIRE(D % 4 == 0, "critic_scores: D must be a multiple of 4");
    BG_REQUIRE(lde % 4 == 0 && ((reinterpret_cast<uintptr_t>(embed) | reinterpret_cast<uintptr_t>(w)) & 15) == 0,
               "critic_scores: 16-byte loads need lde %% 4 == 0 (got %d) and 16-byte aligned embed / w", lde);
    hipLaunchKernelGGL(critic_scores_kernel, dim3(cdiv(rows, 4)), dim3(256), 0, s, embed, lde, w, b, u, noise_scale, frac, scores, (long)rows, D, seed, iter, status_current());
    LAUNCH_CHECK();
}

__device__ __forceinline__ void ar_pick_tail(const ArPickTail& t, const int* d_step, long row, long token, int lane) {
    if (!t.out_all) return;
    const long j = t.fwd_idx[*d_step];
    if (lane == 0) t.out_all[row * t.N + j] = token;
    if (!t.x) return;
    const long id = token < 0 ? 0 : (token >= t.vocab_rows ? t.vocab_rows - 1 : token);
    const float4* te = reinterpret_cast<const float4*>(t.tok_emb + id * t.D);
    const float4* ie = reinterpret_cast<const float4*>(t.img_embed ? t.img_embed + (row * t.C * t.T + j) * t.D : t.tok_emb);
    const float4* pe = reinterpret_cast<const float4*>(t.pos_emb + j * t.D);
    float4* xo = reinterpret_cast<float4*>(t.x + row * t.D);
    const int nv = t.D >> 2;
    for (int o0 = 0; o0 < nv; o0 += 256) {
        float4 a[4], b[4], c[4];
#pragma unroll
        for (int k = 0; k < 4; ++k) {
            const int o = min(o0 + lane + 64 * k, nv - 1);
            a[k] = te[o]; b[k] = ie[o]; c[k] = pe[o];
        }
#pragma unroll
        for (int k = 0; k < 4; ++k) {
            const int o = o0 + lane + 64 * k;
            if (o < nv) {
                const float f = t.img_embed ? 1.f : 0.f;
                xo[o] = make_float4((a[k].x + f * b[k].x) + c[k].x, (a[k].y + f * b[k].y) + c[k].y, (a[k].z + f * b[k].z) + c[k].z, (a[k].w + f * b[k].w) + c[k].w);
            }
        }
    }
}

__global__ __launch_bounds__(64) void ar_pick_kernel(const float* __restrict__ logits, int ldl, const float* __restrict__ u_base, const int* __restrict__ d_step,
                                                     const int64_t* __restrict__ forced, int64_t* __restrict__ out, int V, int top_k, float temperature, ArPickTail tail,
                                                     unsigned* __restrict__ status) {
    const int lane = threadIdx.x;
    const long row = blockIdx.x;
    if (forced) {
        const int64_t f = forced[(d_step ? (long)(*d_step) * gridDim.x : 0) + row];
        if (f >= 0) {
            if (lane == 0) out[row] = f;
            ar_pick_tail(tail, d_step, row, f, lane);
            return;
        }
    }
    const float* u = u_base ? u_base + (d_step ? (long)(*d_step) * gridDim.x : 0) : nullptr;
    const float* lr = logits + row * ldl;
    const int per = (V + 63) / 64;
    float x[VPL_MAX];
    uint32_t key[VPL_MAX];
    bool valid[VPL_MAX];
#pragma unroll
    for (int j = 0; j < VPL_MAX; ++j) {
        const int i = lane * per + j;
        valid[j] = j < per && i < V;
        const float raw = valid[j] ? lr[i] : 0.f;
        if (nonfinite(raw)) status_raise(status, BG_ST_NONFINITE_LOGITS);
        x[j] = valid[j] ? raw / temperature : -INFINITY;
        key[j] = ordered_key(x[j]);
    }
    if (top_k > 0 && top_k < V) {
        const uint32_t thr = kth_largest_key(key, valid, top_k);
#pragma unroll
        for (int j = 0; j < VPL_MAX; ++j)
            if (valid[j] && key[j] < thr) x[j] = -INFINITY;
    }
    float mx = -INFINITY;
    int midx = 0x7fffffff;
#pragma unroll
    for (int j = 0; j < VPL_MAX; ++j)
        if (valid[j] && x[j] > mx) { mx = x[j]; midx = lane * per + j; }
    wave_argmax(mx, midx);
    if (!u) {
        if (lane == 0) out[row] = midx;
        ar_pick_tail(tail, d_step, row, midx, lane);
        return;
    }
    float e[VPL_MAX], local = 0.f;
#pragma unroll
    for (int j = 0; j < VPL_MAX; ++j) {
        e[j] = valid[j] ? expf(x[j] - mx) : 0.f;
        local += e[j];
    }
    float incl = local;
#pragma unroll
    for (int o = 1; o < 64; o <<= 1) {
        const float t = __shfl_up(incl, o, 64);
        if (lane >= o) incl += t;
    }
    const float total = __shfl(incl, 63, 64);
    const float target = u[row] * total;
    float run = incl - local;
    int cand = 0x7fffffff, last = -1;
#pragma unroll
    for (int j = 0; j < VPL_MAX; ++j) {
        if (!valid[j]) continue;
        run += e[j];
        if (e[j] > 0.f) {
            last = lane * per + j;
            if (run > target && cand == 0x7fffffff) cand = lane * per + j;
        }
    }
#pragma unroll
    for (int o = 32; o > 0; o >>= 1) {
        cand = min(cand, __shfl_xor(cand, o, 64));
        last = max(last, __shfl_xor(last, o, 64));
    }
    const int picked = cand != 0x7fffffff ? cand : last;
    if (lane == 0) out[row] = picked;
    ar_pick_tail(tail, d_step, row, picked, lane);
}

void launch_ar_pick(const float* logits, int ldl, const float* u, const int* d_step, const int64_t* forced, int64_t* out, int rows, int V, int top_k, float temperature,
                    hipStream_t s, const ArPickTail* tail) {
    BG_REQUIRE(V <= 64 * VPL_MAX, "ar_pick: vocabulary %d > %d", V, 64 * VPL_MAX);
    BG_REQUIRE(!tail || !tail->out_all || d_step, "ar_pick: the fused tail reads the step from the device counter");
    BG_REQUIRE(!tail || !tail->x || tail->D % 4 == 0, "ar_pick: the fused embedding needs D %% 4 == 0");
    hipLaunchKernelGGL(ar_pick_kernel, dim3(rows), dim3(64), 0, s, logits, ldl, u, d_step, forced, out, V, top_k, temperature, tail ? *tail : ArPickTail{}, status_current());
    LAUNCH_CHECK();
}

constexpr int SCORE_V4 = 8;
template <bool REG>
__global__ __launch_bounds__(256) void ar_score_rows_kernel(const float* __restrict__ logits, int ldl, const int64_t* __restrict__ target, const float* __restrict__ weight,
                                                            const int64_t* __restrict__ fwd_idx, long b, int s0, int rows, int N, int V, float* __restrict__ nll,
                                                            float* __restrict__ wnll, unsigned* __restrict__ status) {
    const int lane = threadIdx.x & 63;
    const int r = blockIdx.x * 4 + (threadIdx.x >> 6);
    if (r >= rows) return;
    const float* lr = logits + (long)r * ldl;
    bool nf = false;
    float mx = -INFINITY, sum = 0.f;
    if (REG) {
        const float4* l4 = reinterpret_cast<const float4*>(lr);
        const int nv = V >> 2;
        float4 v[SCORE_V4];
#pragma unroll
        for (int k = 0; k < SCORE_V4; ++k) {
            const int o = lane + 64 * k;
            v[k] = o < nv ? l4[o] : make_float4(-INFINITY, -INFINITY, -INFINITY, -INFINITY);
            if (o < nv) nf = nf || nonfinite(v[k].x) || nonfinite(v[k].y) || nonfinite(v[k].z) || nonfinite(v[k].w);
            mx = fmaxf(fmaxf(mx, fmaxf(v[k].x, v[k].y)), fmaxf(v[k].z, v[k].w));
        }
        mx = wave_max(mx);
#pragma unroll
        for (int k = 0; k < SCORE_V4; ++k)
            if (lane + 64 * k < nv) sum += (expf(v[k].x - mx) + expf(v[k].y - mx)) + (expf(v[k].z - mx) + expf(v[k].w - mx));
    } else {
        for (int i = lane; i < V; i += 64) {
            const float x = lr[i];
            nf = nf || nonfinite(x);
            mx = fmaxf(mx, x);
        }
        mx = wave_max(mx);
        for (int i = lane; i < V; i += 64) sum += expf(lr[i] - mx);
    }
    sum = wave_sum(sum);
    if (nf) status_raise(status, BG_ST_NONFINITE_LOGITS);
    if (!target || lane != 0) return;
    const int s = s0 + r;
    const long j = fwd_idx[s];
    const long t = target[b * N + j];
    const float v = (t >= 0 && t < V) ? (mx + logf(sum)) - lr[t] : __uint_as_float(0x7fc00000u);
    if (nll) nll[r] = v;
    wnll[r] = weight ? weight[b * N + j] * v : v;
}
void launch_ar_score_rows(const float* logits, int ldl, const int64_t* target, const float* weight, const int64_t* fwd_idx, int b, int s0, int rows, int N, int V,
                          float* nll, float* wnll, hipStream_t s) {
    BG_REQUIRE(rows >= 1 && s0 >= 0 && s0 + rows <= N, "ar_score_rows: decode positions [%d, %d) outside [0, %d)", s0, s0 + rows, N);
    BG_REQUIRE(!target || wnll, "ar_score_rows: a target needs the weighted-nll buffer");
    const bool reg = V % 4 == 0 && ldl % 4 == 0 && V <= 64 * 4 * SCORE_V4 && (reinterpret_cast<uintptr_t>(logits) & 15) == 0;
    if (reg) hipLaunchKernelGGL(ar_score_rows_kernel<true>, dim3(cdiv(rows, 4)), dim3(256), 0, s, logits, ldl, target, weight, fwd_idx, (long)b, s0, rows, N, V, nll, wnll, status_current());
    else hipLaunchKernelGGL(ar_score_rows_kernel<false>, dim3(cdiv(rows, 4)), dim3(256), 0, s, logits, ldl, target, weight, fwd_idx, (long)b, s0, rows, N, V, nll, wnll, status_current());
    LAUNCH_CHECK();
}

__global__ __launch_bounds__(256) void mean_fixed_order_kernel(const float* __restrict__ x, long n, float* __restrict__ out) {
    __shared__ double sh[256];
    double acc = 0.0;
    for (long i = threadIdx.x; i < n; i += 256) acc += (double)x[i];
    sh[threadIdx.x] = acc;
    __syncthreads();
    for (int o = 128; o > 0; o >>= 1) {
        if ((int)threadIdx.x < o) sh[threadIdx.x] += sh[threadIdx.x + o];
        __syncthreads();
    }
    if (threadIdx.x == 0) out[0] = (float)(sh[0] / (double)n);
}
void launch_mean_fixed_order(const float* x, long n, float* out, hipStream_t s) {
    hipLaunchKernelGGL(mean_fixed_order_kernel, dim3(1), dim3(256), 0, s, x, n, out);
    LAUNCH_CHECK();
}

__global__ void philox_fill_kernel(float* __restrict__ out, long n, unsigned long long seed, unsigned iter, unsigned stream, int V) {
    for (long i = (long)blockIdx.x * blockDim.x + threadIdx.x; i < n; i += (long)gridDim.x * blockDim.x) {
        if (stream == 0 && V > 0) {
            unsigned long long block; int word;
            philox_gumbel_block(i / V, V, (int)(i % V), block, word);
            out[i] = philox_to_unit(philox4(seed, block, iter, 0u).v[word]);
        } else {
            out[i] = philox_uniform(seed, (unsigned long long)i, iter, stream);
        }
    }
}
void launch_philox_fill(float* out, long n, unsigned long long seed, unsigned iter, unsigned stream, int V, hipStream_t s) {
    hipLaunchKernelGGL(philox_fill_kernel, dim3((int)std::min<long>((n + 255) / 256, 8192)), dim3(256), 0, s, out, n, seed, iter, stream, V);
    LAUNCH_CHECK();
}

}
```

Baseline: 11.20 scenes/s.

## Compact the final MaskGit transformer layer to masked token rows only

In the last transformer layer of the generator pass, only rows whose tokens are still masked are carried forward. A rowmap kernel lists those rows, and their activations and per-row packed attention biases are gathered. The Q projection, attention, output projection, cross-attention and FFN, logits GEMM and pick then run on this reduced row set, with the pick scattering results back through the rowmap. Keys and values still come from all tokens. This cuts the final-layer and logits work in late iterations where few tokens stay masked, at the cost of extra gather and bias-packing launches, a serial per-sequence rank scan, and more workspace.

```diff
diff --git a/bevgen_amd/csrc/attention_split.hip b/bevgen_amd/csrc/attention_split.hip
--- a/bevgen_amd/csrc/attention_split.hip
+++ b/bevgen_amd/csrc/attention_split.hip
@@ -57,7 +57,7 @@
     const int ntiles_all = a.Nk_pad / SKT;
     const int t_first = KS ? ks * ntiles_all / nks : 0;
     const int ntiles = KS ? (ks + 1) * ntiles_all / nks - t_first : ntiles_all;
-    const float* Bp = a.bias_pk + (long)head * a.bias_head_stride + (long)(qblk * 8 + wave) * a.bias_pk_qb_stride + lane * 4 + (long)t_first * bstep;
+    const float* Bp = a.bias_pk + (long)b * a.bias_batch_stride + (long)head * a.bias_head_stride + (long)(qblk * 8 + wave) * a.bias_pk_qb_stride + lane * 4 + (long)t_first * bstep;
 
     half8 qh[4], qs[4], qls[4];
 #pragma unroll
@@ -119,7 +119,7 @@
         for (int r = 0; r < 16; ++r) bacc[r] = (float)(lane + r);
         rh = make_uint4(lane, 1, 2, 3); rl = rh;
     }
-    const float* Bu = a.bias_pk + (long)head * a.bias_head_stride + (long)(qblk * 8 + wave_u) * a.bias_pk_qb_stride + (long)t_first * bstep;
+    const float* Bu = a.bias_pk + (long)b * a.bias_batch_stride + (long)head * a.bias_head_stride + (long)(qblk * 8 + wave_u) * a.bias_pk_qb_stride + (long)t_first * bstep;
     const __amdgpu_buffer_rsrc_t rs_b = __builtin_amdgcn_make_buffer_rsrc(const_cast<float*>(Bu), 0, -1, 0x00020000);
     auto gload_bias = [&](int tile) {
         if (BEVGEN_ATTN_DIAG & (2 | 8)) return;
@@ -347,11 +347,30 @@
     const int q = min(32 * qb + (lane & 31), Nq - 1);
     reinterpret_cast<float4*>(out)[i] = *reinterpret_cast<const float4*>(bias + (long)q * ld + 32 * tile + 8 * g + 4 * (lane >> 5));
 }
+__global__ __launch_bounds__(256) void pack_attn_bias_rows_kernel(const float* __restrict__ bias, int ld, const int32_t* __restrict__ rowmap, int N, int Nq, int ntiles,
+                                                                  float* __restrict__ out, long per4, long total4) {
+    const long i = (long)blockIdx.x * 256 + threadIdx.x;
+    if (i >= total4) return;
+    const long b = i / per4, ii = i - b * per4;
+    const int lane = (int)(ii & 63), g = (int)((ii >> 6) & 3);
+    const long t = ii >> 8;
+    const int tile = (int)(t % ntiles), qb = (int)(t / ntiles);
+    const int q = min(32 * qb + (lane & 31), Nq - 1);
+    const int row = min(max(rowmap[b * Nq + q] - (int)b * N, 0), N - 1);
+    reinterpret_cast<float4*>(out)[i] = *reinterpret_cast<const float4*>(bias + (long)row * ld + 32 * tile + 8 * g + 4 * (lane >> 5));
+}
 long attn_bias_packed_floats(int Nq, int Nk_pad) { return (long)cdiv(Nq, 256) * 8 * (Nk_pad / SKT) * 1024; }
 void launch_pack_attn_bias(const float* bias, int ld, int Nq, int Nk_pad, float* out, hipStream_t s) {
     BG_REQUIRE(Nk_pad % SKT == 0 && Nk_pad > 0 && ld % 4 == 0 && ld >= Nk_pad, "pack_attn_bias: Nk_pad=%d ld=%d", Nk_pad, ld);
     const long total4 = attn_bias_packed_floats(Nq, Nk_pad) / 4;
     hipLaunchKernelGGL(pack_attn_bias_kernel, dim3((unsigned)cdiv(total4, 256L)), dim3(256), 0, s, bias, ld, Nq, Nk_pad / SKT, out, total4);
+    LAUNCH_CHECK();
+}
+
+void launch_pack_attn_bias_rows(const float* bias, int ld, const int32_t* rowmap, int B, int N, int Nq, int Nk_pad, float* out, hipStream_t s) {
+    BG_REQUIRE(Nk_pad % SKT == 0 && Nk_pad > 0 && ld % 4 == 0 && ld >= Nk_pad && Nq >= 1 && Nq <= N && B >= 1, "pack_attn_bias_rows: Nq=%d N=%d Nk_pad=%d ld=%d", Nq, N, Nk_pad, ld);
+    const long per4 = attn_bias_packed_floats(Nq, Nk_pad) / 4, total4 = per4 * B;
+    hipLaunchKernelGGL(pack_attn_bias_rows_kernel, dim3((unsigned)cdiv(total4, 256L)), dim3(256), 0, s, bias, ld, rowmap, N, Nq, Nk_pad / SKT, out, per4, total4);
     LAUNCH_CHECK();
 }
 
@@ -410,7 +429,7 @@
     a.bias_pk_qb_stride = (long)(a.Nk_pad / SKT) * 1024;
     if (a.bias_pk == nullptr) {
         a.bias_pk = zero_block();
-        a.bias_head_stride = 0; a.bias_pk_tile_step = 0; a.bias_pk_qb_stride = 0;
+        a.bias_head_stride = 0; a.bias_pk_tile_step = 0; a.bias_pk_qb_stride = 0; a.bias_batch_stride = 0;
     }
     const dim3 grid(cdiv(a.Nq, 256), a.H, a.B * a.ksplit);
     ProfScope prof(PROF_ATTN, 4.0 * a.B * a.H * (double)a.Nq * a.Nk_pad * 64, s);
diff --git a/bevgen_amd/csrc/kernels.h b/bevgen_amd/csrc/kernels.h
--- a/bevgen_amd/csrc/kernels.h
+++ b/bevgen_amd/csrc/kernels.h
@@ -135,11 +135,13 @@
     int ksplit = 1;
     float* kws = nullptr;
     unsigned* status = nullptr;
+    long bias_batch_stride = 0;
 };
 constexpr int kAttnPartPitch = 68;
 inline long attn_split_ws_floats(int B, int H, int Nq, int ksplit) { return (long)ksplit * B * H * Nq * kAttnPartPitch; }
 long attn_bias_packed_floats(int Nq, int Nk_pad);
 void launch_pack_attn_bias(const float* bias, int ld, int Nq, int Nk_pad, float* out, hipStream_t s);
+void launch_pack_attn_bias_rows(const float* bias, int ld, const int32_t* rowmap, int B, int N, int Nq, int Nk_pad, float* out, hipStream_t s);
 void launch_attn_split_operands(const float* q, const float* k, const float* v, void* Qh, void* Ql, void* Kh, void* Kl, void* VTh, void* VTl, int B, int H, int Nq, int Nk_pad,
                                 float qmul, hipStream_t s);
 void launch_attention_split(const AttnSplitArgs& a, hipStream_t s);
@@ -293,7 +295,10 @@
 void launch_remask(int64_t* ids, const float* scores, const int64_t* init_ids , int rows, int T, int n_mask, int64_t mask_id, hipStream_t s);
 void launch_maskgit_pick(int64_t* ids, const float* logits, int ldl, const float* gumbel_u , int rows, int V, int k, float temperature,
                          int64_t mask_id, hipStream_t s, unsigned long long seed = 0 , unsigned iter = 0,
-                         float* conf_scores = nullptr, int conf_mode = 0 );
+                         float* conf_scores = nullptr, int conf_mode = 0 ,
+                         const int32_t* rowmap = nullptr );
+void launch_maskgit_rowmap(const int64_t* ids, int32_t* rowmap, int seqs, int T, int n_mask, int64_t mask_id, hipStream_t s);
+void launch_gather_rows2(const int32_t* rowmap, const float* a, float* out_a, const float* b, float* out_b, int rows, int D, hipStream_t s);
 void launch_critic_scores(const float* embed, int lde, const float* w, const float* b, const float* u , float noise_scale, float frac,
                           float* scores, int rows, int D, hipStream_t s, unsigned long long seed = 0, unsigned iter = 0);
 void launch_philox_fill(float* out, long n, unsigned long long seed, unsigned iter, unsigned stream, int V , hipStream_t s);
diff --git a/bevgen_amd/csrc/muse.cpp b/bevgen_amd/csrc/muse.cpp
--- a/bevgen_amd/csrc/muse.cpp
+++ b/bevgen_amd/csrc/muse.cpp
@@ -48,6 +48,8 @@
     const int ks = std::min(std::min(4, (int)(256 / blocks)), ntiles / 8);
     return std::max(ks, 1);
 }
+
+constexpr double kCompactMaxFrac = 0.95;
 
 size_t muse_ws_bytes(const Ctx& c, int B) {
     const size_t rows = (size_t)B * c.N;
@@ -68,7 +70,8 @@
         if (ks > 1) f += (size_t)attn_split_ws_floats(B, c.H, c.N, ks);
     }
     f += rows * (size_t)(2 * (c.D / 32) + 2 * (c.Fpad / 32) + 4);
-    return f * sizeof(float) + (64 + 4 * c.cfg.num_layers) * 256 + (rows <= kSkMaxRows ? gemm_sk_ws_bytes() + 256 : 0);
+    f += rows + (size_t)B * (attn_bias_packed_floats(c.N, c.NkS_pad) + attn_bias_packed_floats(c.N, c.NkC_pad));
+    return f * sizeof(float) + (68 + 4 * c.cfg.num_layers) * 256 + (rows <= kSkMaxRows ? gemm_sk_ws_bytes() + 256 : 0);
 }
 
 void gemm(const float* A, int lda, const float* W, int ldb, float* C, int ldc, int M, int N, int K, const float* R, int ldr, hipStream_t s) {
@@ -94,24 +97,26 @@
 }
 
 void gemm_planes(const void* Aplanes, int lda, const float* W, int ldb, float* C, int ldc, int M, int N, int K, const float* R, int ldr, hipStream_t s, float* kpart = nullptr,
-                 const LnFold* fold = nullptr, MuseWs* sk = nullptr) {
+                 const LnFold* fold = nullptr, MuseWs* sk = nullptr, long plan_rows = 0 ) {
     GemmArgs g;
     g.A_hi = reinterpret_cast<const uint16_t*>(Aplanes); g.A_lo = g.A_hi + 32;
     g.B = W; g.C = C; g.R = R;
     g.M = M; g.N = N; g.K = K;
     g.lda = lda; g.ldb = ldb; g.ldc = ldc; g.ldr = ldr;
-    const bool use_sk = sk && gemm_sk_pays(M, N, K);
-    if (kpart && N <= 1024 && !fold && !use_sk) { g.ksplit = pick_ksplit(M, N, K); g.kpart = kpart; }
+    if (plan_rows <= 0) plan_rows = M;
+    const bool use_sk = sk && gemm_sk_pays(plan_rows, N, K);
+    if (kpart && N <= 1024 && !fold && !use_sk) { g.ksplit = pick_ksplit(plan_rows, N, K); g.kpart = kpart; }
     set_fold(g, fold, M);
     if (use_sk) set_sk(g, sk);
     launch_gemm(g, s);
 }
 
 void gemm_planes_q(const void* Aplanes, int lda, const float* W, const float* q_scale, void* Qh, void* Ql, int B, int H, int Nq, int D, hipStream_t s, float* kpart = nullptr,
-                   float* qraw = nullptr, const LnFold* fold = nullptr, MuseWs* sk = nullptr) {
-    const bool use_sk = sk && gemm_sk_pays((long)B * Nq, H * 64, D);
-    if (!fold && !use_sk && kpart && qraw && H * 64 <= 1024 && pick_ksplit((long)B * Nq, H * 64, D) > 1) {
-        gemm_planes(Aplanes, lda, W, D, qraw, H * 64, B * Nq, H * 64, D, nullptr, 0, s, kpart);
+                   float* qraw = nullptr, const LnFold* fold = nullptr, MuseWs* sk = nullptr, long plan_rows = 0) {
+    if (plan_rows <= 0) plan_rows = (long)B * Nq;
+    const bool use_sk = sk && gemm_sk_pays(plan_rows, H * 64, D);
+    if (!fold && !use_sk && kpart && qraw && H * 64 <= 1024 && pick_ksplit(plan_rows, H * 64, D) > 1) {
+        gemm_planes(Aplanes, lda, W, D, qraw, H * 64, B * Nq, H * 64, D, nullptr, 0, s, kpart, nullptr, nullptr, plan_rows);
         launch_muse_q_prep_split(qraw, q_scale, Qh, Ql, B, H, Nq, 8.0f * kLog2e, s);
         return;
     }
@@ -213,7 +218,21 @@
     }
 }
 
-void muse_blocks(Ctx& c, MuseWs& w, const int64_t* ids, hipStream_t s) {
+struct CompactTail {
+    int Nc = 0;
+    const int32_t* rowmap = nullptr;
+    float *bias_self = nullptr, *bias_cross = nullptr;
+    float *x = nullptr, *xn = nullptr;
+};
+
+struct TailRows {
+    int B = 0, Nq = 0, rows = 0;
+    float *x = nullptr, *xn = nullptr;
+    const float *bias_self_pk = nullptr, *bias_cross_pk = nullptr; long bias_self_bs = 0, bias_cross_bs = 0;
+    MuseWs* sk = nullptr;
+};
+
+float* muse_blocks(Ctx& c, MuseWs& w, const int64_t* ids, hipStream_t s, const CompactTail* ct = nullptr) {
     const auto& g = c.cfg;
     const std::string p = "transformer.";
     const int D = c.D, H = c.H, B = w.B, N = c.N;
@@ -221,31 +240,47 @@
     launch_token_embed(ids, c.pf(p + "token_emb.weight"), w.img, c.pf(p + "pos_emb.weight"), w.x, B, N, D, g.vocab_size + 1, s);
     const bool split = g.precision == BEVGEN_PRECISION_F16X3;
     const int fold = split ? ln_fold_level(c, rows) : 0;
+    BG_REQUIRE(!ct || (split && fold <= 1 && ct->Nc >= 1 && ct->Nc <= N), "muse_blocks: the compact tail needs the split precision and LayerNorm fold level 0 or 1");
     bool x_planes_ready = false;
     const char* merge_env = getenv("BEVGEN_LN_MERGE");
     const bool tile_merge = merge_env ? merge_env[0] == 't' : rows <= 3072;
-    auto consumer = [&](const float* gsums, int groups, int count, const float* cs) {
+    auto consumer = [&](const float* gsums, int groups, int count, const float* cs, int nrows) {
         LnFold f;
         f.in_cs = cs;
         if (tile_merge) { f.in_gsums = gsums; f.in_groups = groups; f.in_count = count; }
-        else { launch_ln_stats_finalize(gsums, w.rowstat, rows, groups, count, 1e-5f, s); f.in_stats = w.rowstat; }
+        else { launch_ln_stats_finalize(gsums, w.rowstat, nrows, groups, count, 1e-5f, s); f.in_stats = w.rowstat; }
         return f;
     };
     LnFold prod_x;
     prod_x.out_planes = w.xn; prod_x.out_stats = w.stats_d; prod_x.out_ld = D;
+    TailRows full;
+    full.B = B; full.Nq = N; full.rows = rows; full.x = w.x; full.xn = w.xn; full.bias_self_pk = c.bias_self_pk; full.bias_cross_pk = c.bias_cross_pk; full.sk = &w;
+    TailRows R = full;
     for (int i = 0; i < g.num_layers; ++i) {
         const MuseLayer& l = c.muse[i];
+        const bool cl = ct && i + 1 == g.num_layers;
+        R = full;
+        if (cl) {
+            R.Nq = ct->Nc; R.rows = B * ct->Nc; R.x = ct->x; R.xn = ct->xn; R.sk = nullptr;
+            R.bias_self_pk = ct->bias_self; R.bias_self_bs = attn_bias_packed_floats(ct->Nc, c.NkS_pad);
+            R.bias_cross_pk = ct->bias_cross; R.bias_cross_bs = attn_bias_packed_floats(ct->Nc, c.NkC_pad);
+        }
         if (split) {
             const bool f0 = fold == 2 && x_planes_ready;
             LnFold cons_x;
             if (!f0) launch_layernorm_planes(w.x, D, l.norm_g[0], nullptr, w.xn, D, rows, D, 1e-5f, s);
-            else cons_x = consumer(w.stats_d, D / 32, D, nullptr);
+            else cons_x = consumer(w.stats_d, D / 32, D, nullptr, rows);
+            if (cl) {
+                launch_gather_rows2(ct->rowmap, w.xn, ct->xn, w.x, ct->x, R.rows, D, s);
+                launch_pack_attn_bias_rows(c.bias_self, c.ldS, ct->rowmap, B, N, ct->Nc, c.NkS_pad, ct->bias_self, s);
+                launch_pack_attn_bias_rows(c.bias_cross, c.ldC, ct->rowmap, B, N, ct->Nc, c.NkC_pad, ct->bias_cross, s);
+            }
             static const int qkv_merge = getenv("BEVGEN_QKV_MERGE") ? atoi(getenv("BEVGEN_QKV_MERGE")) : 1;
-            const bool merged = l.to_qkv_self && qkv_merge != 0 && (qkv_merge != 3 || rows <= 3072);
+            const bool merged = l.to_qkv_self && qkv_merge != 0 && (qkv_merge != 3 || rows <= 3072) && !cl;
             if (!merged) {
                 cons_x.in_cs = l.fold_q_self_cs;
-                gemm_planes_q(w.xn, D, f0 ? l.fold_q_self : l.to_q[0], l.q_scale[0], w.Q, reinterpret_cast<_Float16*>(w.Q) + (size_t)rows * D, B, H, N, D, s, w.kpart, w.qraw,
-                              f0 ? &cons_x : nullptr, &w);
+                gemm_planes_q(R.xn, D, f0 ? l.fold_q_self : l.to_q[0], l.q_scale[0], w.Q, reinterpret_cast<_Float16*>(w.Q) + (size_t)R.rows * D, B, H, R.Nq, D, s, w.kpart, w.qraw,
+                              f0 ? &cons_x : nullptr, R.sk, rows);
             }
             {
                 const size_t kvS_ = (size_t)B * H * c.NkS_pad * 64;
@@ -272,14 +307,15 @@
             gemm(w.xn, D, l.to_q[0], D, w.qraw, D, rows, D, D, nullptr, 0, s);
             gemm(w.xn, D, l.to_kv[0], D, w.kvraw, 2 * D, rows, 2 * D, D, nullptr, 0, s);
         }
-        const size_t qN = (size_t)rows * D, kvS = (size_t)B * H * c.NkS_pad * 64, kvC = (size_t)(B / w.S) * H * c.NkC_pad * 64;
+        const int Nq = R.Nq, trows = R.rows;
+        const size_t qN = (size_t)trows * D, kvS = (size_t)B * H * c.NkS_pad * 64, kvC = (size_t)(B / w.S) * H * c.NkC_pad * 64;
         _Float16 *Qh = reinterpret_cast<_Float16*>(w.Q), *Ksh = reinterpret_cast<_Float16*>(w.Ks), *VTsh = reinterpret_cast<_Float16*>(w.Vs);
         AttnSplitArgs sa{};
         if (split) {
             sa.Qh = Qh; sa.Ql = Qh + qN; sa.Kh = Ksh; sa.Kl = Ksh + kvS; sa.VTh = VTsh; sa.VTl = VTsh + kvS;
-            sa.bias = c.bias_self; sa.bias_pk = c.bias_self_pk; sa.O = w.att; sa.B = B; sa.H = H; sa.Nq = N; sa.Nk_pad = c.NkS_pad;
+            sa.bias = c.bias_self; sa.bias_pk = R.bias_self_pk; sa.bias_batch_stride = R.bias_self_bs; sa.O = w.att; sa.B = B; sa.H = H; sa.Nq = Nq; sa.Nk_pad = c.NkS_pad;
             sa.ldbias = c.ldS; sa.bias_head_stride = 0; sa.scale = 8.0f * kLog2e;
-            sa.o_bstride = (long)N * D; sa.o_qstride = D; sa.o_hstride = 64;
+            sa.o_bstride = (long)Nq * D; sa.o_qstride = D; sa.o_hstride = 64;
             sa.Op = reinterpret_cast<_Float16*>(w.att);
             sa.ksplit = w.attn_ks; sa.kws = w.attn_ws;
             launch_attention_split(sa, s);
@@ -296,14 +332,14 @@
         a.ldbias = c.ldS; a.bias_head_stride = 0; a.scale = 8.0f;
         a.o_bstride = (long)N * D; a.o_qstride = D; a.o_hstride = 64;
         if (!split) launch_attention(a, s);
-        if (split) gemm_planes(w.att, D, l.to_out[0], D, w.x, D, rows, D, D, w.x, D, s, w.kpart, fold == 2 ? &prod_x : nullptr, &w);
+        if (split) gemm_planes(w.att, D, l.to_out[0], D, R.x, D, trows, D, D, R.x, D, s, w.kpart, fold == 2 ? &prod_x : nullptr, R.sk, rows);
         else gemm(w.att, D, l.to_out[0], D, w.x, D, rows, D, D, w.x, D, s);
         if (split) {
             LnFold cons_x;
-            if (fold != 2) launch_layernorm_planes(w.x, D, l.norm_g[1], nullptr, w.xn, D, rows, D, 1e-5f, s);
-            else cons_x = consumer(w.stats_d, D / 32, D, l.fold_q_cross_cs);
-            gemm_planes_q(w.xn, D, fold == 2 ? l.fold_q_cross : l.to_q[1], l.q_scale[1], w.Q, reinterpret_cast<_Float16*>(w.Q) + (size_t)rows * D, B, H, N, D, s, w.kpart, w.qraw,
-                          fold == 2 ? &cons_x : nullptr, &w);
+            if (fold != 2) launch_layernorm_planes(R.x, D, l.norm_g[1], nullptr, R.xn, D, trows, D, 1e-5f, s);
+            else cons_x = consumer(w.stats_d, D / 32, D, l.fold_q_cross_cs, trows);
+            gemm_planes_q(R.xn, D, fold == 2 ? l.fold_q_cross : l.to_q[1], l.q_scale[1], w.Q, reinterpret_cast<_Float16*>(w.Q) + qN, B, H, Nq, D, s, w.kpart, w.qraw,
+                          fold == 2 ? &cons_x : nullptr, R.sk, rows);
         } else {
             launch_layernorm(w.x, D, l.norm_g[1], nullptr, w.xn, D, rows, D, 1e-5f, s);
             gemm(w.xn, D, l.to_q[1], D, w.qraw, D, rows, D, D, nullptr, 0, s);
@@ -311,7 +347,7 @@
         if (split) {
             _Float16 *ckh = reinterpret_cast<_Float16*>(w.crossK[i]), *cvh = reinterpret_cast<_Float16*>(w.crossV[i]);
             sa.Kh = ckh; sa.Kl = ckh + kvC; sa.VTh = cvh; sa.VTl = cvh + kvC;
-            sa.bias = c.bias_cross; sa.bias_pk = c.bias_cross_pk; sa.Nk_pad = c.NkC_pad; sa.ldbias = c.ldC;
+            sa.bias = c.bias_cross; sa.bias_pk = R.bias_cross_pk; sa.bias_batch_stride = R.bias_cross_bs; sa.Nk_pad = c.NkC_pad; sa.ldbias = c.ldC;
             sa.kv_group = w.S;
             launch_attention_split(sa, s);
         } else {
@@ -323,32 +359,32 @@
             launch_attention(a, s);
         }
         if (split) {
-            gemm_planes(w.att, D, l.to_out[1], D, w.x, D, rows, D, D, w.x, D, s, w.kpart, fold == 2 ? &prod_x : nullptr, &w);
-            if (fold != 2) launch_layernorm_planes(w.x, D, l.ff_g0, nullptr, w.xn, D, rows, D, 1e-5f, s);
+            gemm_planes(w.att, D, l.to_out[1], D, R.x, D, trows, D, D, R.x, D, s, w.kpart, fold == 2 ? &prod_x : nullptr, R.sk, rows);
+            if (fold != 2) launch_layernorm_planes(R.x, D, l.ff_g0, nullptr, R.xn, D, trows, D, 1e-5f, s);
             if (l.ff_w1_geglu) {
                 GemmArgs ge;
-                ge.A_hi = reinterpret_cast<const uint16_t*>(w.xn); ge.A_lo = ge.A_hi + 32;
+                ge.A_hi = reinterpret_cast<const uint16_t*>(R.xn); ge.A_lo = ge.A_hi + 32;
                 ge.B = fold == 2 ? l.fold_w1 : l.ff_w1_geglu; ge.C = w.h;
-                ge.M = rows; ge.N = 2 * c.Fpad; ge.K = D;
+                ge.M = trows; ge.N = 2 * c.Fpad; ge.K = D;
                 ge.lda = D; ge.ldb = D; ge.ldc = c.Fpad;
                 ge.epi = EPI_GEGLU;
                 LnFold fg;
-                if (fold == 2) fg = consumer(w.stats_d, D / 32, D, l.fold_w1_cs);
+                if (fold == 2) fg = consumer(w.stats_d, D / 32, D, l.fold_w1_cs, trows);
                 if (fold >= 1) { fg.out_planes = w.g; fg.out_stats = w.stats_f; fg.out_ld = c.Fpad; }
-                if (fold >= 1) set_fold(ge, &fg, rows);
-                if (gemm_sk_pays(rows, ge.N, ge.K)) set_sk(ge, &w);
+                if (fold >= 1) set_fold(ge, &fg, trows);
+                if (R.sk && gemm_sk_pays(rows, ge.N, ge.K)) set_sk(ge, R.sk);
                 launch_gemm(ge, s);
-                if (fold == 0) launch_layernorm_planes(w.h, c.Fpad, l.ff_g3, nullptr, w.g, c.Fpad, rows, c.F, 1e-5f, s);
+                if (fold == 0) launch_layernorm_planes(w.h, c.Fpad, l.ff_g3, nullptr, w.g, c.Fpad, trows, c.F, 1e-5f, s);
             } else {
-                gemm_planes(w.xn, D, l.ff_w1, D, w.h, 2 * c.F, rows, 2 * c.F, D, nullptr, 0, s);
-                launch_geglu_layernorm_planes(w.h, 2 * c.F, l.ff_g3, w.g, c.Fpad, rows, c.F, 1e-5f, s);
+                gemm_planes(R.xn, D, l.ff_w1, D, w.h, 2 * c.F, trows, 2 * c.F, D, nullptr, 0, s);
+                launch_geglu_layernorm_planes(w.h, 2 * c.F, l.ff_g3, w.g, c.Fpad, trows, c.F, 1e-5f, s);
             }
             LnFold fd;
-            if (fold >= 1 && l.ff_w1_geglu) fd = consumer(w.stats_f, c.Fpad / 32, c.F, l.fold_w4_cs);
+            if (fold >= 1 && l.ff_w1_geglu) fd = consumer(w.stats_f, c.Fpad / 32, c.F, l.fold_w4_cs, trows);
             const bool prod_next = fold == 2 && i + 1 < g.num_layers;
             if (prod_next) { fd.out_planes = w.xn; fd.out_stats = w.stats_d; fd.out_ld = D; }
             const bool cons = fd.in_stats || fd.in_gsums, any = cons || fd.out_planes;
-            gemm_planes(w.g, c.Fpad, cons ? l.fold_w4 : l.ff_w4_padded, c.Fpad, w.x, D, rows, D, c.Fpad, w.x, D, s, w.kpart, any ? &fd : nullptr, &w);
+            gemm_planes(w.g, c.Fpad, cons ? l.fold_w4 : l.ff_w4_padded, c.Fpad, R.x, D, trows, D, c.Fpad, R.x, D, s, w.kpart, any ? &fd : nullptr, R.sk, rows);
             x_planes_ready = prod_next;
         } else {
             gemm(w.att, D, l.to_out[1], D, w.x, D, rows, D, D, w.x, D, s);
@@ -358,7 +394,8 @@
             gemm(w.g, c.Fpad, l.ff_w4_padded, c.Fpad, w.x, D, rows, D, c.Fpad, w.x, D, s);
         }
     }
-    launch_layernorm(w.x, D, c.pf(p + "transformer_blocks.norm.gamma"), nullptr, w.xn, D, rows, D, 1e-5f, s);
+    launch_layernorm(R.x, D, c.pf(p + "transformer_blocks.norm.gamma"), nullptr, R.xn, D, R.rows, D, 1e-5f, s);
+    return R.xn;
 }
 
 }
@@ -368,7 +405,7 @@
     BG_REQUIRE(B >= 1, "batch must be positive");
     MuseWs w;
     muse_prepare(c, w, cond, I_inv, E_inv, B, s);
-    muse_blocks(c, w, ids, s);
+    (void)muse_blocks(c, w, ids, s);
     const int rows = (int)w.rows;
     if (embed) HIP_CHECK(hipMemcpyAsync(embed, w.xn, (size_t)rows * c.D * sizeof(float), hipMemcpyDeviceToDevice, s));
     if (logits) gemm(w.xn, c.D, c.pf("transformer.to_logits.weight"), c.D, logits, c.V, rows, c.V, c.D, nullptr, 0, s);
@@ -390,18 +427,52 @@
     float* scores = c.arena.get<float>((size_t)rows);
     const int64_t mask_id = c.cfg.vocab_size;
     int64_t* ids = out;
+    const char* cenv = getenv("BEVGEN_MASKGIT_COMPACT");
+    const char* fenv = getenv("BEVGEN_MASKGIT_COMPACT_MAX");
+    const double cmax = fenv ? atof(fenv) : kCompactMaxFrac;
+    const bool split = c.cfg.precision == BEVGEN_PRECISION_F16X3;
+    const bool compact_ok = (cenv ? atoi(cenv) != 0 : true) && split && score_mode == 0 && !init_ids && ln_fold_level(c, rows) <= 1 && !gemm_sk_pays(rows, D, D) &&
+                            !gemm_sk_pays(rows, 2 * c.Fpad, D) && !gemm_sk_pays(rows, 2 * D, D);
+    auto masked_per_seq = [&](int step) { return step == 0 ? T : std::max(0, std::min((int)sched[step], T)); };
+    auto takes_compact = [&](int step) {
+        const long mc = (long)seqs * masked_per_seq(step);
+        return compact_ok && mc >= 1 && mc < rows && (double)mc <= cmax * (double)rows;
+    };
+    CompactTail ct;
+    int32_t* rowmap = nullptr;
+    {
+        int nmax = 0;
+        for (int step = 0; step < timesteps; ++step)
+            if (takes_compact(step)) nmax = std::max(nmax, masked_per_seq(step));
+        if (nmax > 0) {
+            const int ncmax = c.cfg.num_cams * nmax;
+            rowmap = c.arena.get<int32_t>((size_t)seqs * nmax);
+            ct.bias_self = c.arena.get<float>((size_t)B * attn_bias_packed_floats(ncmax, c.NkS_pad));
+            ct.bias_cross = c.arena.get<float>((size_t)B * attn_bias_packed_floats(ncmax, c.NkC_pad));
+            ct.x = w.kvraw; ct.xn = w.kvraw + (size_t)rows * D;
+            ct.rowmap = rowmap;
+        }
+    }
     launch_fill_i64(ids, rows, mask_id, s);
     launch_fill(scores, rows, 0.f, s);
     for (int step = 0; step < timesteps; ++step) {
         const int steps_until_x0 = timesteps - 1 - step;
         const double frac = (double)steps_until_x0 / (double)timesteps;
         launch_remask(ids, scores, init_ids, seqs, T, sched[step], mask_id, s);
-        muse_blocks(c, w, ids, s);
-        gemm(w.xn, D, c.pf("transformer.to_logits.weight"), D, logits, V, rows, V, D, nullptr, 0, s);
-        launch_maskgit_pick(ids, logits, V, gumbel_u ? gumbel_u + (size_t)step * rows * V : nullptr, rows, V, topk_k, (float)((double)temperature * frac), mask_id, s,
-                            noise_seed, (unsigned)step, score_mode ? scores : nullptr, score_mode);
+        const bool compact = takes_compact(step);
+        int lrows = rows;
+        if (compact) {
+            const int n_mask = masked_per_seq(step);
+            ct.Nc = c.cfg.num_cams * n_mask;
+            lrows = seqs * n_mask;
+            launch_maskgit_rowmap(ids, rowmap, seqs, T, n_mask, mask_id, s);
+        }
+        const float* embed = muse_blocks(c, w, ids, s, compact ? &ct : nullptr);
+        gemm(embed, D, c.pf("transformer.to_logits.weight"), D, logits, V, lrows, V, D, nullptr, 0, s);
+        launch_maskgit_pick(ids, logits, V, gumbel_u ? gumbel_u + (size_t)step * rows * V : nullptr, lrows, V, topk_k, (float)((double)temperature * frac), mask_id, s,
+                            noise_seed, (unsigned)step, score_mode ? scores : nullptr, score_mode, compact ? rowmap : nullptr);
         if (score_mode == 0 && step + 1 < timesteps) {
-            muse_blocks(c, w, ids, s);
+            (void)muse_blocks(c, w, ids, s);
             launch_critic_scores(w.xn, D, c.pf("token_critic.to_pred.weight"), c.pf("token_critic.to_pred.bias"),
                                  critic_u ? critic_u + (size_t)step * rows : nullptr, critic_noise_scale, (float)frac, scores, rows, D, s, noise_seed, (unsigned)step);
         }
diff --git a/bevgen_amd/csrc/sampler.hip b/bevgen_amd/csrc/sampler.hip
--- a/bevgen_amd/csrc/sampler.hip
+++ b/bevgen_amd/csrc/sampler.hip
@@ -61,16 +61,18 @@
 
 __global__ __launch_bounds__(256) void maskgit_pick_kernel(int64_t* __restrict__ ids, const float* __restrict__ logits, int ldl, const float* __restrict__ gumbel_u,
                                                            long rows, int V, int k, float temp_div, int64_t mask_id, unsigned long long seed, unsigned iter,
-                                                           float* __restrict__ conf_scores, int conf_mode, unsigned* __restrict__ status) {
+                                                           float* __restrict__ conf_scores, int conf_mode, unsigned* __restrict__ status,
+                                                           const int32_t* __restrict__ rowmap) {
     const int lane = threadIdx.x & 63;
-    const long row = (long)blockIdx.x * 4 + (threadIdx.x >> 6);
-    if (row >= rows) return;
+    const long lrow = (long)blockIdx.x * 4 + (threadIdx.x >> 6);
+    if (lrow >= rows) return;
+    const long row = rowmap ? rowmap[lrow] : lrow;
     const bool was_mask = ids[row] == mask_id;
     if (!was_mask) {
         if (conf_mode == 1 && lane == 0) conf_scores[row] = -1e5f;
         if (conf_mode != 2) return;
     }
-    const float* lr = logits + row * ldl;
+    const float* lr = logits + lrow * ldl;
     float x[VPL_MAX];
     uint32_t key[VPL_MAX];
     bool valid[VPL_MAX];
@@ -129,13 +131,59 @@
 }
 
 void launch_maskgit_pick(int64_t* ids, const float* logits, int ldl, const float* gumbel_u, int rows, int V, int k, float temperature, int64_t mask_id, hipStream_t s,
-                         unsigned long long seed, unsigned iter, float* conf_scores, int conf_mode) {
+                         unsigned long long seed, unsigned iter, float* conf_scores, int conf_mode, const int32_t* rowmap) {
     BG_REQUIRE(V <= 64 * VPL_MAX, "maskgit_pick: vocabulary %d > %d", V, 64 * VPL_MAX);
+    BG_REQUIRE(!rowmap || conf_mode == 0, "maskgit_pick: compact logits rows carry no confidence scores");
+    if (rows <= 0) return;
     BG_REQUIRE(k >= 1, "maskgit_pick: top-k count %d < 1 (topk_filter_thres = 1 keeps no logit)", k);
     BG_REQUIRE(conf_mode == 0 || conf_scores, "maskgit_pick: confidence scores requested without an output buffer");
     const float temp_div = fmaxf(temperature, 1e-10f);
     hipLaunchKernelGGL(maskgit_pick_kernel, dim3(cdiv(rows, 4)), dim3(256), 0, s, ids, logits, ldl, gumbel_u, (long)rows, V, k, temp_div, mask_id, seed, iter, conf_scores,
-                       conf_mode, status_current());
+                       conf_mode, status_current(), rowmap);
+    LAUNCH_CHECK();
+}
+
+__global__ __launch_bounds__(256) void maskgit_rowmap_kernel(const int64_t* __restrict__ ids, int32_t* __restrict__ rowmap, int T, int n_mask, int64_t mask_id) {
+    extern __shared__ float sc[];
+    unsigned char* mk = reinterpret_cast<unsigned char*>(sc);
+    const int seq = blockIdx.x;
+    for (int i = threadIdx.x; i < T; i += blockDim.x) mk[i] = ids[(long)seq * T + i] == mask_id;
+    __syncthreads();
+    int total = 0;
+    for (int j = 0; j < T; ++j) total += mk[j];
+    for (int i = threadIdx.x; i < T; i += blockDim.x) {
+        if (!mk[i]) continue;
+        int rank = 0;
+        for (int j = 0; j < i; ++j) rank += mk[j];
+        if (rank < n_mask) rowmap[(long)seq * n_mask + rank] = seq * T + i;
+    }
+    for (int r = total + threadIdx.x; r < n_mask; r += blockDim.x) rowmap[(long)seq * n_mask + r] = seq * T;
+}
+
+void launch_maskgit_rowmap(const int64_t* ids, int32_t* rowmap, int seqs, int T, int n_mask, int64_t mask_id, hipStream_t s) {
+    BG_REQUIRE(T >= 1 && T <= 64 * 1024 && n_mask >= 1 && n_mask <= T && (long)seqs * T < 0x7fffffffL, "maskgit_rowmap: T=%d n_mask=%d seqs=%d", T, n_mask, seqs);
+    hipLaunchKernelGGL(maskgit_rowmap_kernel, dim3(seqs), dim3(256), (size_t)((T + 3) & ~3), s, ids, rowmap, T, n_mask, mask_id);
+    LAUNCH_CHECK();
+}
+
+__global__ __launch_bounds__(256) void gather_rows2_kernel(const int32_t* __restrict__ rowmap, const float4* __restrict__ a, float4* __restrict__ out_a, const float4* __restrict__ b,
+                                                           float4* __restrict__ out_b, long rows, int D4) {
+    const int lane = threadIdx.x & 63;
+    const long r = (long)blockIdx.x * 4 + (threadIdx.x >> 6);
+    if (r >= rows) return;
+    const long src = rowmap[r];
+    for (int i = lane; i < D4; i += 64) {
+        out_a[r * D4 + i] = a[src * D4 + i];
+        out_b[r * D4 + i] = b[src * D4 + i];
+    }
+}
+
+void launch_gather_rows2(const int32_t* rowmap, const float* a, float* out_a, const float* b, float* out_b, int rows, int D, hipStream_t s) {
+    if (rows <= 0) return;
+    BG_REQUIRE(D % 4 == 0 && ((reinterpret_cast<uintptr_t>(a) | reinterpret_cast<uintptr_t>(b) | reinterpret_cast<uintptr_t>(out_a) | reinterpret_cast<uintptr_t>(out_b)) & 15) == 0,
+               "gather_rows2: rows of %d floats need 16-byte alignment", D);
+    hipLaunchKernelGGL(gather_rows2_kernel, dim3(cdiv(rows, 4)), dim3(256), 0, s, rowmap, reinterpret_cast<const float4*>(a), reinterpret_cast<float4*>(out_a),
+                       reinterpret_cast<const float4*>(b), reinterpret_cast<float4*>(out_b), (long)rows, D / 4);
     LAUNCH_CHECK();
 }
 
```

New measurement: 11.29 scenes/s, median of 6. About the same (+0.8%).
